# yjtang249/MIPSFusion

Measured on AMD Instinct MI355X. Metric: rays*samples/s per GPU, full optimisation iteration (fwd + bwd + pose+map Adam), 4096 rays x 64 samples, 640x480 RGB-D, higher is better.
Workload: dtype f32; decoder products as 3 x bf16 pieces of each fp32 operand, 6 bf16 MFMAs per product, fp32 accumulate; 1 GPU; BASELINE config 2: FastCaMo-synth apartment_2, 1 active submap per GPU, 4096 rays x 64 samples, hash grid 2^19 x 16 x 2, 620x460 synthetic RGB-D; rays=4096, samples_per_ray=64, hash_size=19, parallelism=single gpu

## Files before the change

include/mipsf.h:

```cpp
#ifndef MIPSF_H
#define MIPSF_H

#include <stdint.h>

#ifdef __cplusplus
extern "C" {
#endif

#define MIPSF_MAX_LEVELS 32
#define MIPSF_ABI_VERSION 2

const char* mipsf_last_error(void);
int mipsf_abi_version(void);
int mipsf_device_cu_count(void);

typedef struct mipsf_grid_meta {
    uint32_t n_levels;
    uint32_t n_features;
    uint32_t log2_hashmap_size;
    uint32_t base_resolution;
    float per_level_scale;
    float log2_per_level_scale;
    uint32_t n_params;
    uint32_t offsets[MIPSF_MAX_LEVELS + 1];
    uint32_t resolutions[MIPSF_MAX_LEVELS];
    float scales[MIPSF_MAX_LEVELS];
} mipsf_grid_meta;

#define MIPSF_SIZE_HASHGRID_BWD_SCRATCH 1
#define MIPSF_SIZE_HASHGRID_COUNTER_WORDS 2
#define MIPSF_SIZE_DECODER_PACKED 3
#define MIPSF_SIZE_DECODER_SAVED 4
#define MIPSF_SIZE_DECODER_DACT 5
#define MIPSF_SIZE_DECODER_WGRAD_PARTIAL 6
#define MIPSF_SIZE_DECODER_PACKED16 7
#define MIPSF_SIZE_DECODER_TILE_WORDS 8
#define MIPSF_SIZE_RENDER_PARTIAL 9
#define MIPSF_SIZE_PLACE_POSE_SCRATCH 10
#define MIPSF_SIZE_POSE_RAYS_SCRATCH 11
#define MIPSF_SIZE_HASHGRID_DET_SCRATCH 12
#define MIPSF_SIZE_DECODER_LIVE_LIST 13
uint64_t mipsf_buffer_size(int which, uint32_t n, uint32_t a, uint32_t b, const mipsf_grid_meta* meta_host);

int mipsf_hashgrid_meta_init(mipsf_grid_meta* meta_host, uint32_t n_levels, uint32_t n_features,
                             uint32_t log2_hashmap_size, uint32_t base_resolution, double per_level_scale);

#define MIPSF_FEAT_AOS 0
#define MIPSF_FEAT_LEVEL_MAJOR 1

int mipsf_hashgrid_fwd(const float* x, const float* params, float* out, float* jac, uint32_t M,
                       const mipsf_grid_meta* meta_host, int layout, void* stream);
int mipsf_hashgrid_dx_from_jac(const float* jac, const float* dout, float* dx, const uint32_t* tile_live, uint32_t M,
                               const mipsf_grid_meta* meta_host, int layout, void* stream);
#define MIPSF_HG_DPARAMS_ZERO 1u
#define MIPSF_HG_ROUTED 2u
#define MIPSF_HG_DETERMINISTIC 4u
#define MIPSF_HG_DET_PIECE 512
#define MIPSF_HG_DET_MAX_ITEMS (1ull << 31)
typedef struct mipsf_hashgrid_bwd_args {
    uint32_t struct_size;
    uint32_t M;
    const float* x;
    const float* params;
    const float* dout;
    float* dparams;
    float* dx;
    float* scratch;
    uint32_t* counters;
    const mipsf_grid_meta* meta;
    int feat_layout;
    uint32_t flags;
} mipsf_hashgrid_bwd_args;
int mipsf_hashgrid_bwd(const mipsf_hashgrid_bwd_args* args_host, void* stream);
int mipsf_hashgrid_route(const float* x, float* scratch, uint32_t M, const mipsf_grid_meta* meta_host, void* stream);
int mipsf_hashgrid_indices(const float* x, uint32_t* idx, uint32_t M, const mipsf_grid_meta* meta_host,
                           void* stream);

int mipsf_freq_fwd(const float* x, float* out, uint32_t M, uint32_t n_dims, uint32_t n_freq, void* stream);
int mipsf_freq_bwd(const float* x, const float* dout, float* dx, uint32_t M, uint32_t n_dims,
                   uint32_t n_freq, void* stream);

typedef struct mipsf_decoder_weights {
    const float* w_pts0; const float* b_pts0;
    const float* w_pts2; const float* b_pts2;
    const float* w_rgb0; const float* b_rgb0;
    const float* w_sdf0; const float* b_sdf0;
    const float* w_sdf2; const float* b_sdf2;
} mipsf_decoder_weights;

typedef struct mipsf_decoder_grads {
    float* w_pts0; float* b_pts0; float* w_pts2; float* b_pts2; float* w_rgb0; float* b_rgb0;
    float* w_sdf0; float* b_sdf0; float* w_sdf2; float* b_sdf2;
} mipsf_decoder_grads;

#define MIPSF_PREC_F32 0
#define MIPSF_PREC_F16X3 1
#define MIPSF_PREC_F16 2
#define MIPSF_PREC_BF16X3 3
#define MIPSF_PREC_BF16X6 4

int mipsf_decoder_pack(const mipsf_decoder_weights* w_host_struct, float* packed, void* stream);
int mipsf_decoder_pack_host(const mipsf_decoder_weights* w_host_ptrs, float* packed_host);
int mipsf_decoder_fwd(const float* packed, const float* feat, int feat_layout, const float* x,
                      const float* embed_pos, int pe_mode, float* out, float* saved, uint32_t M, void* stream);
int mipsf_decoder_fwd_sdf(const float* packed, const float* feat, int feat_layout, const float* x,
                          const float* embed_pos, int pe_mode, float* sdf, uint32_t M, void* stream);
int mipsf_decoder_bwd(const float* packed, const float* feat, int feat_layout, const float* x,
                      const float* embed_pos, int pe_mode, const float* out, const float* dout,
                      const float* saved, float* dfeat, float* dx, float* dembed_pos,
                      const mipsf_decoder_grads* grads_host_struct, float* dact, float* partial,
                      uint32_t M, void* stream);
int mipsf_decoder_bwd_chain(const float* packed, int feat_layout, const float* x, int pe_mode,
                            const float* out, const float* dout, const float* saved, float* dfeat, float* dx,
                            float* dembed_pos, float* dact, uint32_t M, void* stream);
int mipsf_decoder_wgrad(const float* feat, int feat_layout, const float* x, const float* embed_pos, int pe_mode,
                        const float* saved, const float* dact, const mipsf_decoder_grads* grads_host_struct,
                        float* partial, int precision, uint32_t M, void* stream);

int mipsf_decoder_pack16(const mipsf_decoder_weights* w_host_struct, float* packed16, int precision, void* stream);
typedef struct mipsf_decoder_fwd16_args {
    uint32_t struct_size;
    uint32_t M;
    const float* packed16;
    const float* feat;
    const float* x;
    float* out;
    float* saved;
    uint32_t* tile_live_clear;
    int feat_layout;
    int precision;
    int sdf_only;
    int lean_record;
    uint32_t packed16_floats;
} mipsf_decoder_fwd16_args;
int mipsf_decoder_fwd16(const mipsf_decoder_fwd16_args* args_host, void* stream);
#define MIPSF_CHAIN_HEADER_CLEAR 1
#define MIPSF_CHAIN_LEAN_DACT 2
#define MIPSF_CHAIN_BF16X6 4
typedef struct mipsf_decoder_chain16_args {
    uint32_t struct_size;
    uint32_t M;
    const float* packed16;
    const float* x;
    const float* out;
    const float* dout;
    const float* saved;
    float* dfeat;
    float* dx;
    float* dact;
    uint32_t* tile_live;
    int feat_layout;
    int flags;
    uint32_t packed16_floats;
    const uint32_t* live_list;
// ... 63 lines not shown
    double* sums;
    float* draw;
} mipsf_render_fwd_args;
int mipsf_render_fwd(const mipsf_render_fwd_args* args_host, void* stream);
int mipsf_loss_finalize_sums(const double* sums, const mipsf_render_cfg* cfg_host, uint32_t N_total, uint32_t S,
                             float* losses, const float* loss_weights, float* loss_total, void* stream);
typedef struct mipsf_render_bwd_args {
    uint32_t struct_size;
    uint32_t N, S, N_norm;
    const float* raw;
    const float* z_vals;
    const float* target_rgb;
    const float* target_d;
    const uint32_t* counts;
    const float* losses;
    const mipsf_render_cfg* cfg;
    const float* g_losses;
    const float* g_total;
    const float* loss_weights;
    const float* g_rgb;
    const float* g_depth;
    float* draw;
    uint32_t flags;
} mipsf_render_bwd_args;
#define MIPSF_RENDER_BWD_KEEP_IF_UNIT 1u
int mipsf_render_bwd(const mipsf_render_bwd_args* args_host, void* stream);
int mipsf_gather_pose_place_fwd(const float* db, uint64_t n_rows, const int64_t* idx, const float* fixed_poses,
                                const float* rot, const float* trans, uint32_t F, uint32_t K, const int64_t* owner,
                                const float* noise, const float* z_uniform, const float* z_near_offsets,
                                const float* z_near_nodepth, const mipsf_render_cfg* cfg_host, float* d_cam, float* rgb,
                                float* depth, float* z_vals, float* xn, uint32_t* counts, uint32_t N, void* stream);
int mipsf_place_pose_bwd(const float* dxn, const float* z_vals, const mipsf_render_cfg* cfg_host, const float* rot, uint32_t F,
                         uint32_t K, const int64_t* owner, const float* d_cam, float* d_rot, float* d_trans, float* scratch,
                         uint32_t N, uint32_t S, int accumulate, void* stream);
int mipsf_rays_bwd(const float* dxn, const float* z_vals, const mipsf_render_cfg* cfg_host, float* d_rays_o,
                   float* d_rays_d, uint32_t N, uint32_t S, void* stream);
int mipsf_normalise_bwd(const float* dxn, const mipsf_render_cfg* cfg_host, float* dpts, uint32_t M,
                        void* stream);

int mipsf_pose_rays_fwd(const float* db, uint64_t n_rows, const int64_t* idx, const float* fixed_poses,
                        const float* rot, const float* trans, uint32_t F, uint32_t K, const int64_t* owner,
                        float* d_cam, float* rgb, float* depth, float* rays_o, float* rays_d, uint32_t N,
                        void* stream);
#define MIPSF_POSE_MATRIX 0
#define MIPSF_POSE_QUATERNION 1
int mipsf_pose_handover(const float* src, int src_kind, float* rot, float* trans, void* stream);
int mipsf_pose_rays_bwd(const float* g_rays_o, const float* g_rays_d, const float* rot, uint32_t F, uint32_t K,
                        const int64_t* owner, const float* d_cam, float* d_rot, float* d_trans, float* scratch,
                        uint32_t N, int accumulate, void* stream);

int mipsf_adam_step(float* param, float* grad, float* exp_avg, float* exp_avg_sq, uint64_t n, float lr,
                    float beta1, float beta2, float eps, float weight_decay, uint32_t step,
                    const float* hyper_dev, int zero_grad, void* stream);
#define MIPSF_ADAM_MAX_GROUPS 8
int mipsf_adam_advance_n(int32_t* const* step_dev, float* const* hyper_dev, const float* lr, const float* beta1,
                         const float* beta2, uint32_t n_groups, void* stream);

#define MIPSF_ADAM_MAX_TENSORS 16
typedef struct mipsf_adam_tensors {
    uint32_t count;
    float* param[MIPSF_ADAM_MAX_TENSORS];
    float* grad[MIPSF_ADAM_MAX_TENSORS];
    float* exp_avg[MIPSF_ADAM_MAX_TENSORS];
    float* exp_avg_sq[MIPSF_ADAM_MAX_TENSORS];
    uint64_t numel[MIPSF_ADAM_MAX_TENSORS];
} mipsf_adam_tensors;
int mipsf_adam_step_multi(const mipsf_adam_tensors* tensors_host_struct, float lr, float beta1, float beta2,
                          float eps, float weight_decay, uint32_t step, const float* hyper_dev, int zero_grad,
                          void* stream);

#define MIPSF_ADAM_SMALL_MAX_NUMEL 16384
typedef struct mipsf_adam_small {
    uint32_t n_groups, n_tensors;
    int32_t* step_dev[MIPSF_ADAM_MAX_GROUPS];
    float* hyper_dev[MIPSF_ADAM_MAX_GROUPS];
    float lr[MIPSF_ADAM_MAX_GROUPS], beta1[MIPSF_ADAM_MAX_GROUPS], beta2[MIPSF_ADAM_MAX_GROUPS];
    float eps[MIPSF_ADAM_MAX_GROUPS], weight_decay[MIPSF_ADAM_MAX_GROUPS];
    float* param[MIPSF_ADAM_MAX_TENSORS];
    float* grad[MIPSF_ADAM_MAX_TENSORS];
    float* exp_avg[MIPSF_ADAM_MAX_TENSORS];
    float* exp_avg_sq[MIPSF_ADAM_MAX_TENSORS];
    uint32_t numel[MIPSF_ADAM_MAX_TENSORS];
    uint32_t group_of[MIPSF_ADAM_MAX_TENSORS];
} mipsf_adam_small;
int mipsf_adam_step_small(const mipsf_adam_small* desc_host_struct, int zero_grad, void* stream);
#define MIPSF_ADAM_TICKET_WORDS 576
int mipsf_adam_step_all(const mipsf_adam_small* desc_host_struct, int zero_grad, uint32_t* ticket, void* stream);

int mipsf_ro_fitness(const float* raw, uint32_t raw_stride, const float* target_d, float trunc,
                     float* mean_masked, uint32_t P, uint32_t n, void* stream);
int mipsf_ro_fitness_sdf(const float* sdf, const float* target_d, float trunc, float* mean_masked, uint32_t P,
                         uint32_t n, int point_major, void* stream);

#define MIPSF_RO_STATE_FLOATS 32
int mipsf_ro_particles(const float* pst, const float* state, const float* rays_d_cam, const float* target_d,
                       const mipsf_render_cfg* cfg_host, float* xn, float* pst7, uint32_t P, uint32_t n,
                       int point_major, void* stream);
int mipsf_ro_update(const float* mean_masked, const float* pst7, float* state, float sdf_weight, float rescale,
                    uint32_t P, void* stream);

int mipsf_gather_rays(const float* db, uint64_t n_rows, const int64_t* idx, uint32_t N, float* rays7, float* d_cam,
                      float* rgb, float* depth, void* stream);

#ifdef __cplusplus
}
#endif
#endif
```

mipsfusion_amd/_lib.py:

```python
from __future__ import annotations

import ctypes as C
import os
from typing import Optional

import torch

_HERE = os.path.dirname(os.path.abspath(__file__))
LIB_PATH = os.environ.get("MIPSF_LIB") or os.path.join(_HERE, "libmipsf_hip.so")
MAX_LEVELS = 32
FEAT_AOS, FEAT_LEVEL_MAJOR = 0, 1
PREC = {"f32": 0, "f16x3": 1, "f16": 2, "bf16x3": 3, "bf16x6": 4}


class GridMeta(C.Structure):
    _fields_ = [("n_levels", C.c_uint32), ("n_features", C.c_uint32), ("log2_hashmap_size", C.c_uint32),
                ("base_resolution", C.c_uint32), ("per_level_scale", C.c_float),
                ("log2_per_level_scale", C.c_float), ("n_params", C.c_uint32),
                ("offsets", C.c_uint32 * (MAX_LEVELS + 1)), ("resolutions", C.c_uint32 * MAX_LEVELS),
                ("scales", C.c_float * MAX_LEVELS)]


class DecoderWeights(C.Structure):
    _fields_ = [(n, C.c_void_p) for n in ("w_pts0", "b_pts0", "w_pts2", "b_pts2", "w_rgb0", "b_rgb0",
                                          "w_sdf0", "b_sdf0", "w_sdf2", "b_sdf2")]


DecoderGrads = DecoderWeights


class RenderCfg(C.Structure):
    _fields_ = [("n_uniform", C.c_uint32), ("n_near", C.c_uint32), ("perturb", C.c_int), ("use_bound", C.c_int),
                ("bound_min", C.c_double * 3), ("bound_max", C.c_double * 3), ("half_len", C.c_double * 3),
                ("norm_factor", C.c_double), ("trunc", C.c_float), ("sc_factor", C.c_float),
                ("depth_trunc", C.c_float), ("rgb_missing_nonzero", C.c_int), ("emd_w", C.c_float)]


def _args(name, fields):
    cls = type(name, (C.Structure,), {"_fields_": [("struct_size", C.c_uint32)] + fields})

    def new(**kw):
        a = cls()
        a.struct_size = C.sizeof(cls)
        for k, v in kw.items():
            setattr(a, k, v)
        return a
    cls.new = staticmethod(new)
    return cls


_VP, _CU, _CI = C.c_void_p, C.c_uint32, C.c_int
HashgridBwdArgs = _args("HashgridBwdArgs", [("M", _CU), ("x", _VP), ("params", _VP), ("dout", _VP), ("dparams", _VP), ("dx", _VP),
                                            ("scratch", _VP), ("counters", _VP), ("meta", C.POINTER(GridMeta)),
                                            ("feat_layout", _CI), ("flags", _CU)])
DecoderFwd16Args = _args("DecoderFwd16Args", [("M", _CU), ("packed16", _VP), ("feat", _VP), ("x", _VP), ("out", _VP), ("saved", _VP),
                                              ("tile_live_clear", _VP), ("feat_layout", _CI), ("precision", _CI),
                                              ("sdf_only", _CI), ("lean_record", _CI), ("packed16_floats", _CU)])
DecoderChain16Args = _args("DecoderChain16Args", [("M", _CU), ("packed16", _VP), ("x", _VP), ("out", _VP), ("dout", _VP),
                                                  ("saved", _VP), ("dfeat", _VP), ("dx", _VP), ("dact", _VP), ("tile_live", _VP),
                                                  ("feat_layout", _CI), ("flags", _CI), ("packed16_floats", _CU),
                                                  ("live_list", _VP)])
DecoderWgrad16Args = _args("DecoderWgrad16Args", [("M", _CU), ("packed16", _VP), ("feat", _VP), ("x", _VP), ("saved", _VP),
                                                  ("dact", _VP), ("tile_live", _VP), ("grads", C.POINTER(DecoderGrads)),
                                                  ("partial", _VP), ("feat_layout", _CI), ("arithmetic", _CI), ("flags", _CU),
                                                  ("packed16_floats", _CU), ("live_list", _VP)])
RenderFwdArgs = _args("RenderFwdArgs", [("N", _CU), ("S", _CU), ("raw", _VP), ("z_vals", _VP), ("target_rgb", _VP), ("target_d", _VP),
                                        ("counts", _VP), ("cfg", C.POINTER(RenderCfg)), ("rgb", _VP), ("depth", _VP),
                                        ("depth_var", _VP), ("disp", _VP), ("acc", _VP), ("weights", _VP), ("losses", _VP),
                                        ("partial", _VP), ("loss_weights", _VP), ("loss_total", _VP), ("ticket", _VP),
                                        ("sums", _VP), ("draw", _VP)])
RenderBwdArgs = _args("RenderBwdArgs", [("N", _CU), ("S", _CU), ("N_norm", _CU), ("raw", _VP), ("z_vals", _VP), ("target_rgb", _VP),
                                        ("target_d", _VP), ("counts", _VP), ("losses", _VP), ("cfg", C.POINTER(RenderCfg)),
                                        ("g_losses", _VP), ("g_total", _VP), ("loss_weights", _VP), ("g_rgb", _VP),
                                        ("g_depth", _VP), ("draw", _VP), ("flags", _CU)])
RENDER_BWD_KEEP_IF_UNIT = 1

(SIZE_HASHGRID_BWD_SCRATCH, SIZE_HASHGRID_COUNTER_WORDS, SIZE_DECODER_PACKED, SIZE_DECODER_SAVED, SIZE_DECODER_DACT,
 SIZE_DECODER_WGRAD_PARTIAL, SIZE_DECODER_PACKED16, SIZE_DECODER_TILE_WORDS, SIZE_RENDER_PARTIAL, SIZE_PLACE_POSE_SCRATCH,
 SIZE_POSE_RAYS_SCRATCH, SIZE_HASHGRID_DET_SCRATCH, SIZE_DECODER_LIVE_LIST) = range(1, 14)
LIVE_HEADER, LIVE_PAD = 16, 0xFFFFFFFF

HG_DPARAMS_ZERO, HG_ROUTED, HG_DETERMINISTIC = 1, 2, 4
HG_DET_PIECE = 512
HG_DET_MAX_ITEMS = 1 << 31
TILE_ORDER_MAX_M = 1 << 27
WGRAD_LEAN_DACT, WGRAD_DETERMINISTIC = 1, 2


ADAM_MAX_TENSORS = 16


class AdamTensors(C.Structure):
    _fields_ = [("count", C.c_uint32), ("param", C.c_void_p * ADAM_MAX_TENSORS), ("grad", C.c_void_p * ADAM_MAX_TENSORS),
                ("exp_avg", C.c_void_p * ADAM_MAX_TENSORS), ("exp_avg_sq", C.c_void_p * ADAM_MAX_TENSORS),
                ("numel", C.c_uint64 * ADAM_MAX_TENSORS)]


ADAM_MAX_GROUPS = 8
ADAM_SMALL_MAX_NUMEL = 16384


class AdamSmall(C.Structure):
    _fields_ = [("n_groups", C.c_uint32), ("n_tensors", C.c_uint32),
                ("step_dev", C.c_void_p * ADAM_MAX_GROUPS), ("hyper_dev", C.c_void_p * ADAM_MAX_GROUPS),
                ("lr", C.c_float * ADAM_MAX_GROUPS), ("beta1", C.c_float * ADAM_MAX_GROUPS),
                ("beta2", C.c_float * ADAM_MAX_GROUPS), ("eps", C.c_float * ADAM_MAX_GROUPS),
                ("weight_decay", C.c_float * ADAM_MAX_GROUPS),
                ("param", C.c_void_p * ADAM_MAX_TENSORS), ("grad", C.c_void_p * ADAM_MAX_TENSORS),
                ("exp_avg", C.c_void_p * ADAM_MAX_TENSORS), ("exp_avg_sq", C.c_void_p * ADAM_MAX_TENSORS),
                ("numel", C.c_uint32 * ADAM_MAX_TENSORS), ("group_of", C.c_uint32 * ADAM_MAX_TENSORS)]


_P = C.c_void_p
_U32, _U64, _I, _F, _D = C.c_uint32, C.c_uint64, C.c_int, C.c_float, C.c_double

SIGNATURES = {
    "mipsf_last_error": (C.c_char_p, []),
    "mipsf_abi_version": (_I, []),
    "mipsf_device_cu_count": (_I, []),
    "mipsf_buffer_size": (_U64, [_I, _U32, _U32, _U32, C.POINTER(GridMeta)]),
    "mipsf_hashgrid_meta_init": (_I, [C.POINTER(GridMeta), _U32, _U32, _U32, _U32, _D]),
    "mipsf_hashgrid_fwd": (_I, [_P, _P, _P, _P, _U32, C.POINTER(GridMeta), _I, _P]),
    "mipsf_hashgrid_dx_from_jac": (_I, [_P, _P, _P, _P, _U32, C.POINTER(GridMeta), _I, _P]),
    "mipsf_hashgrid_bwd": (_I, [C.POINTER(HashgridBwdArgs), _P]),
    "mipsf_hashgrid_route": (_I, [_P, _P, _U32, C.POINTER(GridMeta), _P]),    "mipsf_hashgrid_indices": (_I, [_P, _P, _U32, C.POINTER(GridMeta), _P]),
    "mipsf_freq_fwd": (_I, [_P, _P, _U32, _U32, _U32, _P]),
    "mipsf_freq_bwd": (_I, [_P, _P, _P, _U32, _U32, _U32, _P]),
    "mipsf_decoder_pack": (_I, [C.POINTER(DecoderWeights), _P, _P]),
    "mipsf_decoder_pack_host": (_I, [C.POINTER(DecoderWeights), _P]),
    "mipsf_decoder_fwd": (_I, [_P, _P, _I, _P, _P, _I, _P, _P, _U32, _P]),
    "mipsf_decoder_fwd_sdf": (_I, [_P, _P, _I, _P, _P, _I, _P, _U32, _P]),
    "mipsf_decoder_bwd": (_I, [_P, _P, _I, _P, _P, _I, _P, _P, _P, _P, _P, _P, C.POINTER(DecoderGrads), _P, _P,
                               _U32, _P]),
    "mipsf_decoder_bwd_chain": (_I, [_P, _I, _P, _I, _P, _P, _P, _P, _P, _P, _P, _U32, _P]),
    "mipsf_decoder_wgrad": (_I, [_P, _I, _P, _P, _I, _P, _P, C.POINTER(DecoderGrads), _P, _I, _U32, _P]),
    "mipsf_decoder_pack16": (_I, [C.POINTER(DecoderWeights), _P, _I, _P]),
    "mipsf_decoder_fwd16": (_I, [C.POINTER(DecoderFwd16Args), _P]),
    "mipsf_decoder_bwd_chain16": (_I, [C.POINTER(DecoderChain16Args), _P]),
    "mipsf_decoder_wgrad16": (_I, [C.POINTER(DecoderWgrad16Args), _P]),
    "mipsf_sample_rays": (_I, [_P, _P, _P, _P, _P, _P, _P, C.POINTER(RenderCfg), _P, _P, _P, _U32, _P]),
    "mipsf_normalise_points": (_I, [_P, C.POINTER(RenderCfg), _P, _U32, _P]),
    "mipsf_render_fwd": (_I, [C.POINTER(RenderFwdArgs), _P]),
    "mipsf_loss_finalize_sums": (_I, [_P, C.POINTER(RenderCfg), _U32, _U32, _P, _P, _P, _P]),
    "mipsf_render_bwd": (_I, [C.POINTER(RenderBwdArgs), _P]),
    "mipsf_gather_pose_place_fwd": (_I, [_P, _U64, _P, _P, _P, _P, _U32, _U32, _P, _P, _P, _P, _P, C.POINTER(RenderCfg), _P, _P,
                                         _P, _P, _P, _P, _U32, _P]),
    "mipsf_place_pose_bwd": (_I, [_P, _P, C.POINTER(RenderCfg), _P, _U32, _U32, _P, _P, _P, _P, _P, _U32, _U32, _I, _P]),
    "mipsf_rays_bwd": (_I, [_P, _P, C.POINTER(RenderCfg), _P, _P, _U32, _U32, _P]),
    "mipsf_normalise_bwd": (_I, [_P, C.POINTER(RenderCfg), _P, _U32, _P]),
    "mipsf_pose_rays_fwd": (_I, [_P, _U64, _P, _P, _P, _P, _U32, _U32, _P, _P, _P, _P, _P, _P, _U32, _P]),
    "mipsf_pose_handover": (_I, [_P, _I, _P, _P, _P]),
    "mipsf_pose_rays_bwd": (_I, [_P, _P, _P, _U32, _U32, _P, _P, _P, _P, _P, _U32, _I, _P]),
    "mipsf_adam_step": (_I, [_P, _P, _P, _P, _U64, _F, _F, _F, _F, _F, _U32, _P, _I, _P]),
    "mipsf_adam_advance_n": (_I, [_P, _P, _P, _P, _P, _U32, _P]),
    "mipsf_adam_step_multi": (_I, [C.POINTER(AdamTensors), _F, _F, _F, _F, _F, _U32, _P, _I, _P]),
    "mipsf_adam_step_small": (_I, [C.POINTER(AdamSmall), _I, _P]),
    "mipsf_adam_step_all": (_I, [C.POINTER(AdamSmall), _I, _P, _P]),
    "mipsf_ro_fitness": (_I, [_P, _U32, _P, _F, _P, _U32, _U32, _P]),
    "mipsf_ro_fitness_sdf": (_I, [_P, _P, _F, _P, _U32, _U32, _I, _P]),
    "mipsf_ro_particles": (_I, [_P, _P, _P, _P, C.POINTER(RenderCfg), _P, _P, _U32, _U32, _I, _P]),
    "mipsf_ro_update": (_I, [_P, _P, _P, _F, _F, _U32, _P]),
    "mipsf_gather_rays": (_I, [_P, _U64, _P, _U32, _P, _P, _P, _P, _P]),
}


SIZE_MCUBES_OFFSET_WORDS, SIZE_MCUBES_WELD_SLOTS, SIZE_MCUBES_WELD_WORDS = 20, 21, 22
MCUBES_BLOCK_CELLS = 4096
McubesArgs = _args("McubesArgs", [("X", _CU), ("Y", _CU), ("Z", _CU), ("isovalue", C.c_float), ("truncation", C.c_float),
                                  ("volume", _VP), ("cases", _VP), ("block_offsets", _VP), ("soup", _VP), ("cell_ids", _VP),
                                  ("capacity_tris", _CU)])
McubesWeldArgs = _args("McubesWeldArgs", [("T", _CU), ("soup", _VP), ("scratch", _VP), ("vertices", _VP), ("faces", _VP),
                                          ("counts", _VP), ("max_rounds", _CU)])
COMPACT_SIGNATURES = {
    "mipsf_decoder_live_compact": (_I, [_P, _U32, _P, _P, _P, _I, _P]),
    "mipsf_hashgrid_dx_from_jac_list": (_I, [_P, _P, _P, _P, _U32, C.POINTER(GridMeta), _I, _P]),
    "mipsf_gather_pose_place_fwd_masked": (_I, [_P, _U64, _P, _P, _P, _P, _U32, _U32, _P, _P, _P, _P, _P, C.POINTER(RenderCfg),
                                                _P, _P, _P, _P, _P, _P, _P, _U32, _P]),
    "mipsf_hashgrid_fwd_masked": (_I, [_P, _P, _P, _P, _P, _U32, _U32, C.POINTER(GridMeta), _I, _P]),
    "mipsf_hashgrid_dx_from_jac_masked": (_I, [_P, _P, _P, _P, _P, _P, _U32, _U32, C.POINTER(GridMeta), _I, _P]),
}

MESH_SIGNATURES = {
    "mipsf_mcubes_count": (_I, [C.POINTER(McubesArgs), _P]),
    "mipsf_mcubes_emit": (_I, [C.POINTER(McubesArgs), _P]),
    "mipsf_mcubes_weld": (_I, [C.POINTER(McubesWeldArgs), _P]),
}


FUSE_KF_FLOATS = 16
FUSE_IN_BOX, FUSE_SEEN = 1, 2


class FusePoints(C.Structure):
# ... 386 lines not shown
```

mipsfusion_amd/csrc/elementwise.hip:

```cpp
#include "common.h"

namespace mipsf {

constexpr float PI_F = 3.14159265358979323846f;
constexpr float HALF_PI_F = 1.57079632679489661923f;

__global__ __launch_bounds__(256) void freq_fwd_kernel(const float* __restrict__ x, float* __restrict__ out,
                                                       uint32_t n, uint32_t n_dims, uint32_t n_freq) {
    const uint32_t t = blockIdx.x * blockDim.x + threadIdx.x;
    if (t >= n) return;
    const uint32_t i = t / n_dims, d = t - i * n_dims;
    const float v = x[t];
    float* o = out + ((size_t)i * n_dims + d) * 2 * n_freq;
    for (uint32_t k = 0; k < n_freq; ++k) {
        const float s = ldexpf(v, (int)k);
        o[2 * k] = sinf(fmaf(s, PI_F, 0.0f));
        o[2 * k + 1] = sinf(fmaf(s, PI_F, HALF_PI_F));
    }
}

__global__ __launch_bounds__(256) void freq_bwd_kernel(const float* __restrict__ x, const float* __restrict__ dout,
                                                       float* __restrict__ dx, uint32_t n, uint32_t n_dims,
                                                       uint32_t n_freq) {
    const uint32_t t = blockIdx.x * blockDim.x + threadIdx.x;
    if (t >= n) return;
    const uint32_t i = t / n_dims, d = t - i * n_dims;
    const float v = x[t];
    const float* g = dout + ((size_t)i * n_dims + d) * 2 * n_freq;
    float acc = 0.f;
    for (uint32_t k = 0; k < n_freq; ++k) {
        const float s = ldexpf(v, (int)k);
        const float fpi = ldexpf(1.0f, (int)k) * PI_F;
        acc = acc + g[2 * k] * (fpi * cosf(fmaf(s, PI_F, 0.0f)));
        acc = acc + g[2 * k + 1] * (fpi * cosf(fmaf(s, PI_F, HALF_PI_F)));
    }
    dx[t] = acc;
}

__global__ __launch_bounds__(256) void normalise_kernel(const float* __restrict__ pts, float* __restrict__ xn,
                                                        uint64_t n3, NormCfg nc) {
    const uint64_t t = (uint64_t)blockIdx.x * blockDim.x + threadIdx.x;
    if (t >= n3) return;
    const int d = (int)(t % 3);
    xn[t] = normalise1(pts[t], nc.sub[d], nc.div[d], nc.norm_factor);
}

__global__ __launch_bounds__(256) void normalise_bwd_kernel(const float* __restrict__ dxn, float* __restrict__ dpts,
                                                            uint64_t n3, NormCfg nc) {
    const uint64_t t = (uint64_t)blockIdx.x * blockDim.x + threadIdx.x;
    if (t >= n3) return;
    const int d = (int)(t % 3);
    dpts[t] = (float)(((double)dxn[t] / nc.norm_factor) / nc.div[d]);
}

struct AdamK {
    float lr_over_bc1, beta1, beta2, one_minus_b1, one_minus_b2, inv_sqrt_bc2, eps, wd;
    const float* dev_hyper;
};

__device__ __forceinline__ AdamK resolve(AdamK k) {
    if (k.dev_hyper) {
        k.lr_over_bc1 = k.dev_hyper[0];
        k.inv_sqrt_bc2 = k.dev_hyper[1];
    }
    return k;
}

__global__ void adam_advance_kernel(int* __restrict__ step, float* __restrict__ hyper, float lr, float beta1,
                                    float beta2) {
    if (threadIdx.x == 0 && blockIdx.x == 0) {
        const int t = step[0] + 1;
        step[0] = t;
        const double bc1 = 1.0 - pow((double)beta1, (double)t);
        const double bc2 = 1.0 - pow((double)beta2, (double)t);
        hyper[0] = (float)((double)lr / bc1);
        hyper[1] = (float)(1.0 / sqrt(bc2));
    }
}

struct AdvanceN {
    int* step[MIPSF_ADAM_MAX_GROUPS];
    float* hyper[MIPSF_ADAM_MAX_GROUPS];
    float lr[MIPSF_ADAM_MAX_GROUPS], beta1[MIPSF_ADAM_MAX_GROUPS], beta2[MIPSF_ADAM_MAX_GROUPS];
    uint32_t n;
};
__global__ void adam_advance_n_kernel(AdvanceN a) {
    const uint32_t i = threadIdx.x;
    if (i >= a.n) return;
    const int t = a.step[i][0] + 1;
    a.step[i][0] = t;
    const double bc1 = 1.0 - pow((double)a.beta1[i], (double)t);
    const double bc2 = 1.0 - pow((double)a.beta2[i], (double)t);
    a.hyper[i][0] = (float)((double)a.lr[i] / bc1);
    a.hyper[i][1] = (float)(1.0 / sqrt(bc2));
}

__device__ __forceinline__ void adam1(float& p, float& g, float& m, float& v, const AdamK& k) {
    float gg = g;
    if (k.wd != 0.f) gg = gg + k.wd * p;
    m = m + (gg - m) * k.one_minus_b1;
    v = v * k.beta2 + (k.one_minus_b2 * gg) * gg;
    const float denom = sqrtf(v) * k.inv_sqrt_bc2 + k.eps;
    p = p - k.lr_over_bc1 * (m / denom);
}

template <bool ZERO>
__global__ __launch_bounds__(256) void adam_kernel(float* __restrict__ p, float* __restrict__ g,
                                                   float* __restrict__ m, float* __restrict__ v, uint64_t n,
                                                   AdamK k_in) {
    const AdamK k = resolve(k_in);
    const uint64_t stride = (uint64_t)gridDim.x * blockDim.x;
    const uint64_t n4 = n / 4;
    float4* p4 = reinterpret_cast<float4*>(p);
    float4* g4 = reinterpret_cast<float4*>(g);
    float4* m4 = reinterpret_cast<float4*>(m);
    float4* v4 = reinterpret_cast<float4*>(v);
    for (uint64_t i = (uint64_t)blockIdx.x * blockDim.x + threadIdx.x; i < n4; i += stride) {
        float4 pp = p4[i], gg = g4[i], mm = m4[i], vv = v4[i];
        adam1(pp.x, gg.x, mm.x, vv.x, k);
        adam1(pp.y, gg.y, mm.y, vv.y, k);
        adam1(pp.z, gg.z, mm.z, vv.z, k);
        adam1(pp.w, gg.w, mm.w, vv.w, k);
        p4[i] = pp;
        m4[i] = mm;
        v4[i] = vv;
        if (ZERO) g4[i] = make_float4(0.f, 0.f, 0.f, 0.f);
    }
    for (uint64_t i = n4 * 4 + (uint64_t)blockIdx.x * blockDim.x + threadIdx.x; i < n; i += stride) {
        float pp = p[i], gg = g[i], mm = m[i], vv = v[i];
        adam1(pp, gg, mm, vv, k);
        p[i] = pp;
        m[i] = mm;
        v[i] = vv;
        if (ZERO) g[i] = 0.f;
    }
}

struct AdamMulti {
    float* p[MIPSF_ADAM_MAX_TENSORS];
    float* g[MIPSF_ADAM_MAX_TENSORS];
    float* m[MIPSF_ADAM_MAX_TENSORS];
    float* v[MIPSF_ADAM_MAX_TENSORS];
    uint64_t n[MIPSF_ADAM_MAX_TENSORS];
};

template <bool ZERO>
__global__ __launch_bounds__(256) void adam_multi_kernel(AdamMulti t, AdamK k_in) {
    const AdamK k = resolve(k_in);
    const int ti = blockIdx.y;
    float *p = t.p[ti], *g = t.g[ti], *m = t.m[ti], *v = t.v[ti];
    const uint64_t n = t.n[ti];
    for (uint64_t i = (uint64_t)blockIdx.x * blockDim.x + threadIdx.x; i < n; i += (uint64_t)gridDim.x * blockDim.x) {
        float pp = p[i], gg = g[i], mm = m[i], vv = v[i];
        adam1(pp, gg, mm, vv, k);
        p[i] = pp, m[i] = mm, v[i] = vv;
        if (ZERO) g[i] = 0.f;
    }
}

template <bool ZERO>
__global__ __launch_bounds__(256) void adam_small_kernel(mipsf_adam_small d) {
    __shared__ float hyp[MIPSF_ADAM_MAX_GROUPS][2];
    if (threadIdx.x < d.n_groups) {
        const uint32_t i = threadIdx.x;
        const int t = d.step_dev[i][0] + 1;
        d.step_dev[i][0] = t;
        const double bc1 = 1.0 - pow((double)d.beta1[i], (double)t);
        const double bc2 = 1.0 - pow((double)d.beta2[i], (double)t);
        const float h0 = (float)((double)d.lr[i] / bc1), h1 = (float)(1.0 / sqrt(bc2));
        hyp[i][0] = h0, hyp[i][1] = h1;
        d.hyper_dev[i][0] = h0, d.hyper_dev[i][1] = h1;
    }
    __syncthreads();
    for (uint32_t ti = 0; ti < d.n_tensors; ++ti) {
        const uint32_t gi = d.group_of[ti];
        AdamK k;
        k.lr_over_bc1 = hyp[gi][0], k.inv_sqrt_bc2 = hyp[gi][1];
        k.beta1 = d.beta1[gi], k.beta2 = d.beta2[gi];
        k.one_minus_b1 = (float)(1.0 - (double)d.beta1[gi]), k.one_minus_b2 = (float)(1.0 - (double)d.beta2[gi]);
        k.eps = d.eps[gi], k.wd = d.weight_decay[gi], k.dev_hyper = nullptr;
        float *p = d.param[ti], *g = d.grad[ti], *m = d.exp_avg[ti], *v = d.exp_avg_sq[ti];
        for (uint32_t i = threadIdx.x; i < d.numel[ti]; i += blockDim.x) {
            float pp = p[i], gg = g[i], mm = m[i], vv = v[i];
            adam1(pp, gg, mm, vv, k);
            p[i] = pp, m[i] = mm, v[i] = vv;
            if (ZERO) g[i] = 0.f;
        }
    }
}

__device__ __forceinline__ double powi(double b, int t) {
    double r = 1.0;
    while (t > 0) {
        if (t & 1) r *= b;
        b *= b;
        t >>= 1;
    }
    return r;
}

__device__ __forceinline__ uint32_t adam_key(float lr, float b1, float b2) {
    return __float_as_uint(lr) ^ (__float_as_uint(b1) * 3u) ^ (__float_as_uint(b2) * 7u);
}

struct AdamAllMap {
    uint32_t blk0[MIPSF_ADAM_MAX_TENSORS + 1];
};

template <bool ZERO>
__global__ __launch_bounds__(256) void adam_all_kernel(mipsf_adam_small d, AdamAllMap map, uint32_t* __restrict__ ticket) {
    __shared__ float hyp[2];
    uint32_t ti = 0;
    while (ti + 1 < d.n_tensors && blockIdx.x >= map.blk0[ti + 1]) ++ti;
    const uint32_t gi = d.group_of[ti];
    float *p = d.param[ti], *g = d.grad[ti], *m = d.exp_avg[ti], *v = d.exp_avg_sq[ti];
    const uint64_t n = d.numel[ti];
    const uint32_t nb = map.blk0[ti + 1] - map.blk0[ti], b = blockIdx.x - map.blk0[ti];
    const uint64_t stride = (uint64_t)nb * 256;
    const bool vec = ((((uintptr_t)p | (uintptr_t)g | (uintptr_t)m | (uintptr_t)v) & 15) == 0);
    const uint64_t n4 = vec ? n / 4 : 0;
    float4* p4 = reinterpret_cast<float4*>(p);
    float4* g4 = reinterpret_cast<float4*>(g);
    float4* m4 = reinterpret_cast<float4*>(m);
    float4* v4 = reinterpret_cast<float4*>(v);
    uint64_t i = (uint64_t)b * 256 + threadIdx.x;
    float4 pp, gg, mm, vv;
    if (i < n4) pp = p4[i], gg = g4[i], mm = m4[i], vv = v4[i];
    uint32_t* nexth = ticket + 16u * 33u + 4u * gi;
    if (threadIdx.x == 0) {
        const int t = d.step_dev[gi][0] + 1;
        const uint32_t tag = nexth[0];
        const float h0 = __uint_as_float(nexth[1]), h1 = __uint_as_float(nexth[2]);
        if (tag == (uint32_t)t && nexth[3] == adam_key(d.lr[gi], d.beta1[gi], d.beta2[gi])) {
            hyp[0] = h0, hyp[1] = h1;
        } else {
            const double bc1 = 1.0 - powi((double)d.beta1[gi], t);
            const double bc2 = 1.0 - powi((double)d.beta2[gi], t);
            hyp[0] = (float)((double)d.lr[gi] / bc1), hyp[1] = (float)(1.0 / sqrt(bc2));
        }
    }
    __syncthreads();
    AdamK k;
    k.lr_over_bc1 = hyp[0], k.inv_sqrt_bc2 = hyp[1];
    k.beta1 = d.beta1[gi], k.beta2 = d.beta2[gi];
    k.one_minus_b1 = (float)(1.0 - (double)d.beta1[gi]), k.one_minus_b2 = (float)(1.0 - (double)d.beta2[gi]);
    k.eps = d.eps[gi], k.wd = d.weight_decay[gi], k.dev_hyper = nullptr;
    if (threadIdx.x == 0) {
        const uint32_t sub = blockIdx.x & 31u;
        const uint32_t n_sub = (gridDim.x - sub + 31u) / 32u;
        bool last = false;
        if (__hip_atomic_fetch_add(ticket + 16u * (1u + sub), 1u, __ATOMIC_RELAXED, __HIP_MEMORY_SCOPE_AGENT) == n_sub - 1) {
            __hip_atomic_store(ticket + 16u * (1u + sub), 0u, __ATOMIC_RELAXED, __HIP_MEMORY_SCOPE_AGENT);
            const uint32_t n_master = gridDim.x < 32u ? gridDim.x : 32u;
            last = __hip_atomic_fetch_add(ticket, 1u, __ATOMIC_RELAXED, __HIP_MEMORY_SCOPE_AGENT) == n_master - 1;
        }
        if (last) {
            for (uint32_t q = 0; q < d.n_groups; ++q) {
                const int t = d.step_dev[q][0] + 1;
                d.step_dev[q][0] = t;
                const double b1 = (double)d.beta1[q], b2 = (double)d.beta2[q];
                d.hyper_dev[q][0] = (float)((double)d.lr[q] / (1.0 - powi(b1, t)));
                d.hyper_dev[q][1] = (float)(1.0 / sqrt(1.0 - powi(b2, t)));
                uint32_t* nx = ticket + 16u * 33u + 4u * q;
                nx[1] = __float_as_uint((float)((double)d.lr[q] / (1.0 - powi(b1, t + 1))));
                nx[2] = __float_as_uint((float)(1.0 / sqrt(1.0 - powi(b2, t + 1))));
                nx[3] = adam_key(d.lr[q], d.beta1[q], d.beta2[q]);
                nx[0] = (uint32_t)(t + 1);
            }
            __hip_atomic_store(ticket, 0u, __ATOMIC_RELAXED, __HIP_MEMORY_SCOPE_AGENT);
        }
    }
    if (i < n4) {
        adam1(pp.x, gg.x, mm.x, vv.x, k);
        adam1(pp.y, gg.y, mm.y, vv.y, k);
        adam1(pp.z, gg.z, mm.z, vv.z, k);
        adam1(pp.w, gg.w, mm.w, vv.w, k);
        p4[i] = pp, m4[i] = mm, v4[i] = vv;
        if (ZERO) g4[i] = make_float4(0.f, 0.f, 0.f, 0.f);
    }
    for (uint64_t r = i + stride; r < n4; r += stride) {
        float4 p1 = p4[r], g1 = g4[r], m1 = m4[r], v1 = v4[r];
        asm volatile("" : "+v"(p1.x), "+v"(g1.x), "+v"(m1.x), "+v"(v1.x));
        adam1(p1.x, g1.x, m1.x, v1.x, k);
        adam1(p1.y, g1.y, m1.y, v1.y, k);
        adam1(p1.z, g1.z, m1.z, v1.z, k);
        adam1(p1.w, g1.w, m1.w, v1.w, k);
        p4[r] = p1, m4[r] = m1, v4[r] = v1;
        if (ZERO) g4[r] = make_float4(0.f, 0.f, 0.f, 0.f);
    }
    for (uint64_t q = n4 * 4 + (uint64_t)b * 256 + threadIdx.x; q < n; q += stride) {
        float p1 = p[q], g1 = g[q], m1 = m[q], v1 = v[q];
        adam1(p1, g1, m1, v1, k);
        p[q] = p1, m[q] = m1, v[q] = v1;
        if (ZERO) g[q] = 0.f;
    }
}

__global__ __launch_bounds__(256) void ro_fitness_kernel(const float* __restrict__ raw, uint32_t stride,
                                                         const float* __restrict__ target_d, float trunc,
                                                         float* __restrict__ out, uint32_t P, uint32_t n,
                                                         uint32_t row_p, uint32_t row_j) {
    const uint32_t wave = (blockIdx.x * blockDim.x + threadIdx.x) / MIPSF_WAVE;
    const uint32_t lane = threadIdx.x & (MIPSF_WAVE - 1);
    if (wave >= P) return;
    float acc = 0.f;
    for (uint32_t j = lane; j < n; j += MIPSF_WAVE) {
        const float s = raw[((size_t)wave * row_p + (size_t)j * row_j) * stride + 3] * trunc;
        acc += (target_d[j] > 0.f) ? fabsf(s) : 0.f;
    }
    acc = wave_sum(acc);
    if (lane == 0) out[wave] = acc / (float)n;
}

}

using namespace mipsf;

extern "C" {

int mipsf_freq_fwd(const float* x, float* out, uint32_t M, uint32_t n_dims, uint32_t n_freq, void* stream) {
    if (M == 0) return 0;
    MIPSF_REQUIRE(x && out, "null pointer");
    const uint32_t n = M * n_dims;
    hipLaunchKernelGGL(freq_fwd_kernel, dim3((n + 255) / 256), dim3(256), 0, (hipStream_t)stream, x, out, n, n_dims,
                       n_freq);
    return check_launch("freq_fwd");
}

int mipsf_freq_bwd(const float* x, const float* dout, float* dx, uint32_t M, uint32_t n_dims, uint32_t n_freq,
                   void* stream) {
    if (M == 0) return 0;
    MIPSF_REQUIRE(x && dout && dx, "null pointer");
    const uint32_t n = M * n_dims;
    hipLaunchKernelGGL(freq_bwd_kernel, dim3((n + 255) / 256), dim3(256), 0, (hipStream_t)stream, x, dout, dx, n,
                       n_dims, n_freq);
    return check_launch("freq_bwd");
}

int mipsf_normalise_points(const float* pts, const mipsf_render_cfg* cfg, float* xn, uint32_t M, void* stream) {
    if (M == 0) return 0;
    MIPSF_REQUIRE(pts && cfg && xn, "null pointer");
    const uint64_t n3 = (uint64_t)M * 3;
    hipLaunchKernelGGL(normalise_kernel, dim3((uint32_t)((n3 + 255) / 256)), dim3(256), 0, (hipStream_t)stream, pts,
                       xn, n3, make_norm(*cfg));
    return check_launch("normalise_points");
}
// ... 11 lines not shown
                       const float* dev_hyper) {
    AdamK k;
    const double bc1 = 1.0 - pow((double)beta1, (double)(step ? step : 1));
    const double bc2 = 1.0 - pow((double)beta2, (double)(step ? step : 1));
    k.lr_over_bc1 = (float)((double)lr / bc1);
    k.beta1 = beta1;
    k.beta2 = beta2;
    k.one_minus_b1 = (float)(1.0 - (double)beta1);
    k.one_minus_b2 = (float)(1.0 - (double)beta2);
    k.inv_sqrt_bc2 = (float)(1.0 / sqrt(bc2));
    k.eps = eps;
    k.wd = weight_decay;
    k.dev_hyper = dev_hyper;
    return k;
}

int mipsf_adam_advance_n(int32_t* const* step_dev, float* const* hyper_dev, const float* lr, const float* beta1,
                         const float* beta2, uint32_t n_groups, void* stream) {
    if (n_groups == 0) return 0;
    MIPSF_REQUIRE(step_dev && hyper_dev && lr && beta1 && beta2, "null pointer");
    MIPSF_REQUIRE(n_groups <= MIPSF_ADAM_MAX_GROUPS, "at most %d groups per call", MIPSF_ADAM_MAX_GROUPS);
    AdvanceN a;
    a.n = n_groups;
    for (uint32_t i = 0; i < n_groups; ++i) {
        MIPSF_REQUIRE(step_dev[i] && hyper_dev[i], "null pointer in group %u", i);
        a.step[i] = step_dev[i], a.hyper[i] = hyper_dev[i], a.lr[i] = lr[i], a.beta1[i] = beta1[i], a.beta2[i] = beta2[i];
    }
    hipLaunchKernelGGL(adam_advance_n_kernel, dim3(1), dim3(64), 0, (hipStream_t)stream, a);
    return check_launch("adam_advance_n");
}

int mipsf_adam_step(float* param, float* grad, float* exp_avg, float* exp_avg_sq, uint64_t n, float lr, float beta1,
                    float beta2, float eps, float weight_decay, uint32_t step, const float* hyper_dev,
                    int zero_grad, void* stream) {
    if (n == 0) return 0;
    MIPSF_REQUIRE(param && grad && exp_avg && exp_avg_sq, "null pointer");
    MIPSF_REQUIRE(step >= 1 || hyper_dev, "step must be >= 1 (or hyper_dev given)");
    MIPSF_REQUIRE((((uintptr_t)param | (uintptr_t)grad | (uintptr_t)exp_avg | (uintptr_t)exp_avg_sq) & 15) == 0,
                  "adam buffers must be 16-byte aligned");
    const AdamK k = make_adam(lr, beta1, beta2, eps, weight_decay, step, hyper_dev);
    uint64_t want = (n / 4 + 255) / 256;
    uint32_t blocks = (uint32_t)(want < 1 ? 1 : (want > 2048 ? 2048 : want));
    if (zero_grad)
        hipLaunchKernelGGL(adam_kernel<true>, dim3(blocks), dim3(256), 0, (hipStream_t)stream, param, grad, exp_avg,
                           exp_avg_sq, n, k);
    else
        hipLaunchKernelGGL(adam_kernel<false>, dim3(blocks), dim3(256), 0, (hipStream_t)stream, param, grad, exp_avg,
                           exp_avg_sq, n, k);
    return check_launch("adam_step");
}

int mipsf_adam_step_multi(const mipsf_adam_tensors* t, float lr, float beta1, float beta2, float eps,
                          float weight_decay, uint32_t step, const float* hyper_dev, int zero_grad, void* stream) {
    MIPSF_REQUIRE(t != nullptr, "null tensor table");
    if (t->count == 0) return 0;
    MIPSF_REQUIRE(t->count <= MIPSF_ADAM_MAX_TENSORS, "too many tensors (%u)", t->count);
    MIPSF_REQUIRE(step >= 1 || hyper_dev, "step must be >= 1 (or hyper_dev given)");
    AdamMulti a;
    uint64_t nmax = 0;
    for (uint32_t i = 0; i < MIPSF_ADAM_MAX_TENSORS; ++i) {
        const bool live = i < t->count;
        a.p[i] = live ? t->param[i] : nullptr, a.g[i] = live ? t->grad[i] : nullptr;
        a.m[i] = live ? t->exp_avg[i] : nullptr, a.v[i] = live ? t->exp_avg_sq[i] : nullptr;
        a.n[i] = live ? t->numel[i] : 0;
        if (live) {
            MIPSF_REQUIRE(a.p[i] && a.g[i] && a.m[i] && a.v[i], "null pointer in tensor %u", i);
            nmax = a.n[i] > nmax ? a.n[i] : nmax;
        }
    }
    const AdamK k = make_adam(lr, beta1, beta2, eps, weight_decay, step, hyper_dev);
    uint64_t bx = (nmax + 255) / 256;
    if (bx > 64) bx = 64;
    if (bx < 1) bx = 1;
    const dim3 grid((uint32_t)bx, t->count);
    if (zero_grad) hipLaunchKernelGGL(adam_multi_kernel<true>, grid, dim3(256), 0, (hipStream_t)stream, a, k);
    else hipLaunchKernelGGL(adam_multi_kernel<false>, grid, dim3(256), 0, (hipStream_t)stream, a, k);
    return check_launch("adam_step_multi");
}

int mipsf_adam_step_small(const mipsf_adam_small* d, int zero_grad, void* stream) {
    MIPSF_REQUIRE(d, "null descriptor");
    MIPSF_REQUIRE(d->n_groups >= 1 && d->n_groups <= MIPSF_ADAM_MAX_GROUPS, "bad group count %u", d->n_groups);
    MIPSF_REQUIRE(d->n_tensors >= 1 && d->n_tensors <= MIPSF_ADAM_MAX_TENSORS, "bad tensor count %u", d->n_tensors);
    for (uint32_t i = 0; i < d->n_groups; ++i) MIPSF_REQUIRE(d->step_dev[i] && d->hyper_dev[i], "null pointer in group %u", i);
    for (uint32_t i = 0; i < d->n_tensors; ++i) {
        MIPSF_REQUIRE(d->param[i] && d->grad[i] && d->exp_avg[i] && d->exp_avg_sq[i], "null pointer in tensor %u", i);
        MIPSF_REQUIRE(d->numel[i] <= MIPSF_ADAM_SMALL_MAX_NUMEL && d->group_of[i] < d->n_groups, "tensor %u out of range", i);
    }
    if (zero_grad) hipLaunchKernelGGL(adam_small_kernel<true>, dim3(1), dim3(256), 0, (hipStream_t)stream, *d);
    else hipLaunchKernelGGL(adam_small_kernel<false>, dim3(1), dim3(256), 0, (hipStream_t)stream, *d);
    return check_launch("adam_step_small");
}

int mipsf_adam_step_all(const mipsf_adam_small* d, int zero_grad, uint32_t* ticket, void* stream) {
    MIPSF_REQUIRE(d && ticket, "null pointer");
    MIPSF_REQUIRE(d->n_groups >= 1 && d->n_groups <= MIPSF_ADAM_MAX_GROUPS, "bad group count %u", d->n_groups);
    MIPSF_REQUIRE(d->n_tensors >= 1 && d->n_tensors <= MIPSF_ADAM_MAX_TENSORS, "bad tensor count %u", d->n_tensors);
    for (uint32_t i = 0; i < d->n_groups; ++i) MIPSF_REQUIRE(d->step_dev[i] && d->hyper_dev[i], "null pointer in group %u", i);
    AdamAllMap map;
    const int cus = device_cus();
    if (cus <= 0) return 3;
    const uint64_t budget = (uint64_t)cus * 8;
    uint64_t want_all = 0;
    for (uint32_t i = 0; i < d->n_tensors; ++i) want_all += ((uint64_t)d->numel[i] / 4 + 255) / 256 + 1;
    uint32_t blocks = 0;
    for (uint32_t i = 0; i < d->n_tensors; ++i) {
        MIPSF_REQUIRE(d->param[i] && d->grad[i] && d->exp_avg[i] && d->exp_avg_sq[i], "null pointer in tensor %u", i);
        MIPSF_REQUIRE(d->group_of[i] < d->n_groups, "tensor %u: group out of range", i);
        map.blk0[i] = blocks;
        uint64_t want = ((uint64_t)d->numel[i] / 4 + 255) / 256 + 1;
        if (want_all > budget) want = want * budget / want_all;
        blocks += (uint32_t)(want < 1 ? 1 : want);
    }
    for (uint32_t i = d->n_tensors; i <= MIPSF_ADAM_MAX_TENSORS; ++i) map.blk0[i] = blocks;
    if (zero_grad) hipLaunchKernelGGL(adam_all_kernel<true>, dim3(blocks), dim3(256), 0, (hipStream_t)stream, *d, map, ticket);
    else hipLaunchKernelGGL(adam_all_kernel<false>, dim3(blocks), dim3(256), 0, (hipStream_t)stream, *d, map, ticket);
    return check_launch("adam_step_all");
}

int mipsf_ro_fitness(const float* raw, uint32_t raw_stride, const float* target_d, float trunc, float* mean_masked,
                     uint32_t P, uint32_t n, void* stream) {
    if (P == 0) return 0;
    MIPSF_REQUIRE(raw && target_d && mean_masked, "null pointer");
    MIPSF_REQUIRE(raw_stride >= 4, "raw_stride must cover the sdf column");
    const uint32_t threads = P * MIPSF_WAVE;
    hipLaunchKernelGGL(ro_fitness_kernel, dim3((threads + 255) / 256), dim3(256), 0, (hipStream_t)stream, raw,
                       raw_stride, target_d, trunc, mean_masked, P, n, n, 1u);
    return check_launch("ro_fitness");
}

int mipsf_ro_fitness_sdf(const float* sdf, const float* target_d, float trunc, float* mean_masked, uint32_t P,
                         uint32_t n, int point_major, void* stream) {
    if (P == 0) return 0;
    MIPSF_REQUIRE(sdf && target_d && mean_masked, "null pointer");
    const uint32_t threads = P * MIPSF_WAVE;
    hipLaunchKernelGGL(ro_fitness_kernel, dim3((threads + 255) / 256), dim3(256), 0, (hipStream_t)stream, sdf - 3, 1u,
                       target_d, trunc, mean_masked, P, n, point_major ? 1u : n, point_major ? P : 1u);
    return check_launch("ro_fitness");
}

}
```

mipsfusion_amd/csrc/hashgrid.hip:

```cpp
#include "common.h"
#include "launch.h"
#include "decoder_layout.h"

namespace mipsf {

constexpr uint32_t P1 = 2654435761u;
constexpr uint32_t P2 = 805459861u;
constexpr int HG_BLOCK = 256;

struct Cell {
    uint32_t c[3];
    float f[3];
};

__device__ __forceinline__ Cell locate(const float* __restrict__ x, uint32_t i, float scale) {
    Cell r;
#pragma unroll
    for (int d = 0; d < 3; ++d) {
        const float pos = fmaf(scale, x[3 * (size_t)i + d], 0.5f);
        const float fl = floorf(pos);
        r.c[d] = (uint32_t)(int)fl;
        r.f[d] = pos - fl;
    }
    return r;
}

template <int MODE>
__device__ __forceinline__ uint32_t corner_index(uint32_t cx, uint32_t cy, uint32_t cz, uint32_t res,
                                                 uint32_t size) {
    if (MODE == 0) {
        uint32_t idx = cx + cy * res + cz * res * res;
        if (idx >= size) {
            idx -= size;
            if (idx >= size) idx %= size;
        }
        return idx;
    }
    const uint32_t h = cx ^ (cy * P1) ^ (cz * P2);
    return MODE == 1 ? (h & (size - 1u)) : (h % size);
}

__host__ __device__ inline bool level_is_hashed(uint32_t res, uint32_t size) {
    uint64_t stride = 1;
    for (int d = 0; d < 3; ++d) {
        if (stride > size) break;
        stride *= res;
        stride &= 0xFFFFFFFFull;
    }
    return size < stride;
}

__device__ __forceinline__ int decode_level(uint32_t n_levels, uint32_t nchunk, uint32_t& chunk) {
    const uint32_t b = blockIdx.x;
    const uint32_t xcd = b & 7u;
    const uint32_t j = b >> 3;
    const uint32_t slot = j / nchunk;
    chunk = j - slot * nchunk;
    const uint32_t nslots = (n_levels + 7u) / 8u;
    return (int)(xcd + 8u * (nslots - 1u - slot));
}

template <int MODE>
__device__ __forceinline__ void corner_indices_m(const Cell& cell, uint32_t res, uint32_t size, uint32_t idx[8]) {
#pragma unroll
    for (int c = 0; c < 8; ++c) {
        idx[c] = corner_index<MODE>(cell.c[0] + (c & 1), cell.c[1] + ((c >> 1) & 1), cell.c[2] + ((c >> 2) & 1),
                                    res, size);
    }
}

__device__ __forceinline__ int level_mode(uint32_t res, uint32_t size) {
    if (!level_is_hashed(res, size)) return 0;
    return (size & (size - 1u)) == 0u ? 1 : 2;
}

__device__ __forceinline__ void corner_indices(int mode, const Cell& cell, uint32_t res, uint32_t size,
                                               uint32_t idx[8]) {
    if (mode == 0) corner_indices_m<0>(cell, res, size, idx);
    else if (mode == 1) corner_indices_m<1>(cell, res, size, idx);
    else corner_indices_m<2>(cell, res, size, idx);
}

__device__ __forceinline__ void corner_weights(const Cell& cell, float w[8]) {
#pragma unroll
// ... 27 lines not shown
        s1 = s1 + wgt * (v[right].y - v[left].y);
    }
}

__device__ __forceinline__ bool ray_wants_dx(const uint32_t* __restrict__ ray_mask, uint32_t S, uint32_t i) {
    return ray_mask == nullptr || ray_mask[S == 64u ? i >> 6 : i / S] != 0u;
}

template <int LAYOUT, bool JAC>
__global__ __launch_bounds__(HG_BLOCK) void hashgrid_fwd_kernel(const float* __restrict__ x,
                                                                const float2* __restrict__ table,
                                                                float* __restrict__ out, float* __restrict__ jac,
                                                                uint32_t M, GridLevels g, uint32_t nchunk,
                                                                const uint32_t* __restrict__ ray_mask, uint32_t S) {
    uint32_t chunk;
    const int level = decode_level(g.n_levels, nchunk, chunk);
    if (level >= (int)g.n_levels) return;
    const uint32_t i = chunk * HG_BLOCK + threadIdx.x;
    if (i >= M) return;

    const uint32_t off = g.offsets[level];
    const uint32_t size = g.offsets[level + 1] - off;
    const uint32_t res = g.res[level];
    const Cell cell = locate(x, i, g.scale[level]);
    uint32_t idx[8];
    corner_indices(level_mode(res, size), cell, res, size, idx);
    float w[8];
    corner_weights(cell, w);
    const float2* lvl = table + off;
    float2 v[8];
#pragma unroll
    for (int c = 0; c < 8; ++c) v[c] = lvl[idx[c]];
    float a0 = 0.f, a1 = 0.f;
#pragma unroll
    for (int c = 0; c < 8; ++c) {
        a0 = fmaf(w[c], v[c].x, a0);
        a1 = fmaf(w[c], v[c].y, a1);
    }
    typedef float f32x2_t __attribute__((ext_vector_type(2)));
    f32x2_t* dst = reinterpret_cast<f32x2_t*>(out + feat_index<LAYOUT>(i, level, M, g.n_levels));
    __builtin_nontemporal_store(f32x2_t{a0, a1}, dst);
    if (JAC && ray_wants_dx(ray_mask, S, i)) {
        f32x2_t* j2 = reinterpret_cast<f32x2_t*>(jac) + (size_t)level * 3 * M + i;
#pragma unroll
        for (int d = 0; d < 3; ++d) {
            float s0, s1;
            level_jacobian(cell, v, g.scale[level], d, s0, s1);
            __builtin_nontemporal_store(f32x2_t{s0, s1}, j2 + (size_t)d * M);
        }
    }
}

constexpr int SC_BLOCK = 1024;
#ifndef MIPSF_SC_PLANAR
#define MIPSF_SC_PLANAR 1
#endif
#if MIPSF_SC_PLANAR
#define SC_ACC0(e) (e)
#define SC_ACC1(e) (sc_plane1 + (e))
#else
#define SC_ACC0(e) (2 * (e))
#define SC_ACC1(e) (2 * (e) + 1)
#endif
#ifndef MIPSF_RT_BLOCK
#define MIPSF_RT_BLOCK 512
#endif
constexpr int RT_BLOCK = MIPSF_RT_BLOCK;
#ifndef MIPSF_SC_MAX_SLICE
#define MIPSF_SC_MAX_SLICE 8192
#endif
constexpr uint32_t SC_MAX_SLICE = MIPSF_SC_MAX_SLICE;
#ifndef MIPSF_SC_SLICE_LOG2
#define MIPSF_SC_SLICE_LOG2 13
#endif
constexpr uint32_t SC_SLICE_LOG2 = MIPSF_SC_SLICE_LOG2;
#ifndef MIPSF_SC_PART
#define MIPSF_SC_PART 24576
#endif
#ifndef MIPSF_SC_PART_DENSE
#define MIPSF_SC_PART_DENSE 8192
#endif
#ifndef MIPSF_SC_RUN
#define MIPSF_SC_RUN 4
#endif
#ifndef MIPSF_SC_SKIP_ZERO
#define MIPSF_SC_SKIP_ZERO 1
#endif
constexpr uint32_t SC_PART = MIPSF_SC_PART;
constexpr uint32_t SC_PART_DENSE = MIPSF_SC_PART_DENSE;
constexpr uint32_t SC_PART_MIN = SC_PART < SC_PART_DENSE ? SC_PART : SC_PART_DENSE;
constexpr uint32_t SC_RUN = MIPSF_SC_RUN;
constexpr uint32_t SC_ROUTE_UNR = 4;
constexpr uint32_t SC_MAX_NS = 512;
constexpr uint32_t SC_MAX_BINS = 8192;
#ifndef MIPSF_SC_MASKED_MAX_M
#define MIPSF_SC_MASKED_MAX_M (1u << 24)
#endif
constexpr uint32_t SC_MASKED_MAX_M = MIPSF_SC_MASKED_MAX_M;

struct ScatterPlan {
    uint32_t n_levels;
    uint32_t n_slices[MIPSF_MAX_LEVELS];
    uint32_t slice_entries[MIPSF_MAX_LEVELS];
    uint32_t slice_shift[MIPSF_MAX_LEVELS];
    uint32_t bin0[MIPSF_MAX_LEVELS + 1];
    uint32_t n_bins;
    uint32_t max_items;
    uint32_t max_slice;
    uint32_t dense_bins;
    uint32_t fresh;
    uint32_t fold_launch;
    uint32_t w_count, w_arrive, w_first, w_parts, w_nitems, w_items;
    uint64_t w_records, w_partial, w_end;
};

static ScatterPlan make_plan(const GridLevels& g, uint32_t M) {
    ScatterPlan p = {};
    p.n_levels = g.n_levels;
    uint32_t bins = 0;
    for (uint32_t l = 0; l < g.n_levels; ++l) {
        const uint32_t size = g.offsets[l + 1] - g.offsets[l];
        const bool one = size <= SC_MAX_SLICE;
        const uint32_t ns = one ? 1u : (size + (1u << SC_SLICE_LOG2) - 1) >> SC_SLICE_LOG2;
        p.n_slices[l] = ns;
        p.slice_entries[l] = one ? size : (1u << SC_SLICE_LOG2);
        p.slice_shift[l] = one ? 31u : SC_SLICE_LOG2;
        p.bin0[l] = bins;
        bins += ns;
    }
    p.bin0[g.n_levels] = bins;
    p.n_bins = bins;
    for (uint32_t l = 0; l < g.n_levels; ++l) {
        if (level_is_hashed(g.res[l], g.offsets[l + 1] - g.offsets[l])) break;
        p.dense_bins = p.bin0[l + 1];
    }
    for (uint32_t l = 0; l < g.n_levels; ++l) p.max_slice = p.slice_entries[l] > p.max_slice ? p.slice_entries[l] : p.max_slice;
    const uint64_t max_records = 8ull * g.n_levels * M;
    p.max_items = (uint32_t)((max_records + SC_PART_MIN - 1) / SC_PART_MIN) + bins;
    uint64_t w = 0;
    p.w_count = (uint32_t)w, w += bins;
    p.w_nitems = (uint32_t)w, w += 4;
    p.w_arrive = (uint32_t)w, w += bins;
    p.w_first = (uint32_t)w, w += bins;
    p.w_parts = (uint32_t)w, w += bins;
    w = (w + 3) / 4 * 4;
    p.w_items = (uint32_t)w;
    w = (w + 15) / 16 * 16;
    p.w_records = w, w += (uint64_t)bins * M;
    w = (w + 15) / 16 * 16;
    p.w_partial = w, w += (uint64_t)p.max_items * SC_MAX_SLICE * 2;
    p.w_end = w;
    return p;
}

__global__ void scatter_zero_kernel(uint32_t* __restrict__ ws, uint32_t n) {
    const uint32_t i = blockIdx.x * blockDim.x + threadIdx.x;
    if (i < n) ws[i] = 0u;
}

__device__ __forceinline__ uint32_t ranked_add(uint32_t* cnt, uint32_t s, bool active, bool aggregate) {
    if (!aggregate) return active ? atomicAdd(&cnt[s], 1u) : 0u;
    const uint32_t lane = threadIdx.x & 63u;
    uint32_t rank = 0;
    unsigned long long todo = __ballot(active);
    while (todo) {
        const int leader = __ffsll((long long)todo) - 1;
        const uint32_t s0 = (uint32_t)__shfl((int)s, leader, 64);
        const unsigned long long m = __ballot(active && s == s0);
        uint32_t b = 0;
        if ((int)lane == leader) b = atomicAdd(&cnt[s0], (uint32_t)__popcll(m));
        b = (uint32_t)__shfl((int)b, leader, 64);
        if (active && s == s0) rank = b + (uint32_t)__popcll(m & ((1ull << lane) - 1ull));
        todo &= ~m;
    }
    return rank;
}

__device__ __forceinline__ void route_groups_general(int mode, const Cell& cell, uint32_t res, uint32_t size,
                                                     uint32_t shift, uint32_t (&s)[8], uint32_t (&m)[8]) {
    uint32_t idx[8];
    corner_indices(mode, cell, res, size, idx);
#pragma unroll
    for (int c = 0; c < 8; ++c) s[c] = idx[c] >> shift;
#pragma unroll
    for (int c = 0; c < 8; ++c) {
        bool first = true;
        uint32_t mm = 0;
#pragma unroll
        for (int k = 0; k < 8; ++k) {
            if (k < c) first = first && (s[k] != s[c]);
            mm |= (s[k] == s[c]) ? (1u << k) : 0u;
        }
        m[c] = first ? mm : 0u;
    }
}

// ... 233 lines not shown
    RT_MARK(5);
    __syncthreads();
    RT_MARK(6);
#pragma unroll
    for (uint32_t u = 0; u < SC_ROUTE_UNR; ++u) {
        const uint32_t i = mine[u];
#pragma unroll
        for (int q = 0; q < 8; ++q) {
            if (q == 4 && !__any(mp[u][1] != 0u)) break;
            const uint32_t m = (mp[u][q >> 2] >> (8 * (q & 3))) & 0xffu;
            if (m) {
                const uint32_t sl = (sp[u][q >> 1] >> (16 * (q & 1))) & 0xffffu;
                const uint32_t rk = (rp[u][q >> 1] >> (16 * (q & 1))) & 0xffffu;
                if (MIPSF_SC_STAGE) {
                    const uint32_t p = lstart[sl] + rk;
                    if (p < STAGE_CAP) {
                        stage[p] = masked ? (i | (m << 24)) : i;
                        continue;
                    }
                }
                rec[(size_t)(bin0 + sl) * M + base[sl] + rk] = masked ? (i | (m << 24)) : i;
            }
        }
    }
    RT_MARK(7);
    if (MIPSF_SC_STAGE) {
        __syncthreads();
        RT_MARK(8);
        const uint32_t wave = threadIdx.x >> 6, lane = threadIdx.x & 63u;
        for (uint32_t q = wave; q < ns; q += RT_BLOCK / 64) {
            const uint32_t n = cnt[q], src = lstart[q];
            uint32_t* dstp = rec + (size_t)(bin0 + q) * M + base[q];
            for (uint32_t p = lane; p < n && src + p < STAGE_CAP; p += 64) dstp[p] = stage[src + p];
        }
    }
#ifdef MIPSF_RT_TRACE
    RT_MARK(9);
    for (int q = 2; q < 9; ++q) tr_acc[q] += tr_t[q + 1] - tr_t[q];
    ++tr_levels;
#endif
    }
#ifdef MIPSF_RT_TRACE
    if ((threadIdx.x & 63u) == 0u) {
        unsigned long long* tr = reinterpret_cast<unsigned long long*>(ws + plan.w_end + 64) + (size_t)(blockIdx.x * (RT_BLOCK / 64) + (threadIdx.x >> 6)) * 10;
        for (int q = 0; q < 9; ++q) tr[q] = tr_acc[q];
        tr[9] = (unsigned long long)(group | (tr_levels << 8));
    }
#endif
}
__device__ __forceinline__ uint32_t part_of(const ScatterPlan& plan, uint32_t bin) {
    return bin < plan.dense_bins ? SC_PART_DENSE : SC_PART;
}

#ifndef MIPSF_SC_PUBLISH_WT
#define MIPSF_SC_PUBLISH_WT 1
#endif

template <bool AGENT>
__device__ __forceinline__ float2 fold_entry(const float2* p2, uint32_t parts, float2 cur) {
    float2 a = make_float2(0.f, 0.f);
    for (uint32_t q = 0; q < parts; q += 8) {
        float2 v[8];
#pragma unroll
        for (uint32_t k = 0; k < 8; ++k) {
            v[k] = make_float2(0.f, 0.f);
            if (q + k < parts) {
                if (AGENT) {
                    const unsigned long long u = __hip_atomic_load(
                        reinterpret_cast<const unsigned long long*>(p2 + (size_t)(q + k) * SC_MAX_SLICE), __ATOMIC_RELAXED,
                        __HIP_MEMORY_SCOPE_AGENT);
                    v[k] = make_float2(__uint_as_float((uint32_t)u), __uint_as_float((uint32_t)(u >> 32)));
                } else {
                    v[k] = p2[(size_t)(q + k) * SC_MAX_SLICE];
                }
            }
        }
#pragma unroll
        for (uint32_t k = 0; k < 8; ++k) a.x += v[k].x, a.y += v[k].y;
    }
    cur.x += a.x, cur.y += a.y;
    return cur;
}

template <int LAYOUT>
__device__ __forceinline__ void scatter_item(const float* __restrict__ x, const float* __restrict__ dout,
                                             float* __restrict__ dparams, uint32_t M, const GridLevels& g,
                                             const ScatterPlan& plan, uint32_t* __restrict__ ws, uint32_t* __restrict__ cw,
                                             uint32_t* sh_flag, double* __restrict__ acc,
                                             const uint4 desc, const uint32_t item_index) {
    const uint32_t item = desc.x;
    const uint32_t sc_plane1 = plan.max_slice;
    (void)sc_plane1;
    const uint32_t bin = item & 0xffffu, part = item >> 16;
    const bool single = desc.z == 1u;
    uint32_t level = 0;
    while (level + 1 < plan.n_levels && bin >= plan.bin0[level + 1]) ++level;
    const uint32_t slice = bin - plan.bin0[level];
    const uint32_t off = g.offsets[level];
    const uint32_t size = g.offsets[level + 1] - off;
    const uint32_t se = plan.slice_entries[level];
    const uint32_t begin = slice * se;
    const uint32_t count = begin + se <= size ? se : size - begin;
    const uint32_t res = g.res[level];
    const float scale = g.scale[level];
    const uint32_t n_rec_bin = desc.y;
    const uint32_t r0 = part * part_of(plan, bin);
    const uint32_t n_rec = n_rec_bin - r0 < part_of(plan, bin) ? n_rec_bin - r0 : part_of(plan, bin);
    const uint32_t* __restrict__ rec = ws + plan.w_records + (size_t)bin * M + r0;

    {
#if MIPSF_SC_PLANAR
        for (uint32_t e = threadIdx.x; e < count; e += SC_BLOCK) acc[SC_ACC0(e)] = 0.0, acc[SC_ACC1(e)] = 0.0;
#else
        double2* z = reinterpret_cast<double2*>(acc);
        for (uint32_t e = threadIdx.x; e < count; e += SC_BLOCK) z[e] = make_double2(0.0, 0.0);
#endif
    }
    float2* dst = reinterpret_cast<float2*>(dparams) + off + begin;
    constexpr uint32_t FL = SC_MAX_SLICE / SC_BLOCK;
    float2 cur[FL];
    if (single && !plan.fresh) {
#pragma unroll
        for (uint32_t k = 0; k < FL; ++k) {
            const uint32_t e = threadIdx.x + k * SC_BLOCK;
            cur[k] = e < count ? dst[e] : make_float2(0.f, 0.f);
        }
    }
    __syncthreads();

    const int mode = level_mode(res, size);
    const bool masked = M <= SC_MASKED_MAX_M;
    uint32_t cc[3] = {0u, 0u, 0u};
    float sum[8][2];
    bool open = false;
    auto flush = [&]() {
#ifdef MIPSF_SC_ABL_DENSE_NOATOM
        if (mode == 0) { asm volatile("" :: "v"(sum[0][0]), "v"(sum[7][1])); return; }
#endif
        Cell cell;
        cell.c[0] = cc[0], cell.c[1] = cc[1], cell.c[2] = cc[2];
        uint32_t idx[8];
        corner_indices(mode, cell, res, size, idx);
        uint32_t hit = 0;
#pragma unroll
        for (int c = 0; c < 8; ++c) {
            idx[c] -= begin;
            hit |= (idx[c] < count) ? (1u << c) : 0u;
        }
        if (mode == 0) {
#pragma unroll
            for (int c = 0; c < 8; ++c) {
                if (hit >> c & 1u) {
                    atomicAdd(&acc[SC_ACC0(idx[c])], (double)sum[c][0]);
                    atomicAdd(&acc[SC_ACC1(idx[c])], (double)sum[c][1]);
                }
            }
            return;
        }
        while (hit) {
            const int c = __ffs((int)hit) - 1;
            hit &= hit - 1u;
            uint32_t e = idx[0];
            float v0 = sum[0][0], v1 = sum[0][1];
#pragma unroll
            for (int k = 1; k < 8; ++k) {
                e = (c == k) ? idx[k] : e;
                v0 = (c == k) ? sum[k][0] : v0;
                v1 = (c == k) ? sum[k][1] : v1;
            }
            atomicAdd(&acc[SC_ACC0(e)], (double)v0);
            atomicAdd(&acc[SC_ACC1(e)], (double)v1);
        }
    };
    if (mode != 0) {
        constexpr int UD = 4;
        for (uint32_t r = threadIdx.x; r < n_rec; r += UD * SC_BLOCK) {
            uint32_t si[UD];
            float px[UD][3];
            float2 pg[UD];
#pragma unroll
            for (int u = 0; u < UD; ++u) {
                const uint32_t q = r + u * SC_BLOCK;
                si[u] = rec[q < n_rec ? q : n_rec - 1];
            }
#pragma unroll
            for (int u = 0; u < UD; ++u) {
                const uint32_t ii = masked ? (si[u] & 0xffffffu) : si[u];
#ifdef MIPSF_SC_ABL_NOGATHER
                px[u][0] = (float)(ii & 1023u) * (1.0f / 1024.0f), px[u][1] = (float)((ii >> 10) & 1023u) * (1.0f / 1024.0f);
                px[u][2] = (float)((ii >> 5) & 1023u) * (1.0f / 1024.0f);
                pg[u] = make_float2(1e-3f, 2e-3f);
#else
                px[u][0] = x[3 * (size_t)ii], px[u][1] = x[3 * (size_t)ii + 1], px[u][2] = x[3 * (size_t)ii + 2];
                pg[u] = *reinterpret_cast<const float2*>(dout + feat_index<LAYOUT>(ii, level, M, g.n_levels));
#endif
            }
#pragma unroll
            for (int u = 0; u < UD; ++u) {
                if (r + u * SC_BLOCK >= n_rec) break;
                Cell cell;
#pragma unroll
                for (int d = 0; d < 3; ++d) {
                    const float pos = fmaf(scale, px[u][d], 0.5f);
                    const float fl = floorf(pos);
// ... 27 lines not shown
                            const float wgt = (cell.f[0] * wy) * wz;
                            atomicAdd(&acc[SC_ACC0(e)], (double)(wgt * gy.x));
                            atomicAdd(&acc[SC_ACC1(e)], (double)(wgt * gy.y));
                        }
                    }
                    continue;
                }
                while (hit) {
                    const int c = __ffs((int)hit) - 1;
                    hit &= hit - 1u;
                    const uint32_t cx = cell.c[0] + (c & 1), cy = cell.c[1] + ((c >> 1) & 1), cz = cell.c[2] + ((c >> 2) & 1);
                    const uint32_t e = (mode == 1 ? corner_index<1>(cx, cy, cz, res, size) : corner_index<2>(cx, cy, cz, res, size)) - begin;
                    float wgt = (c & 1) ? cell.f[0] : 1.0f - cell.f[0];
                    wgt = wgt * ((c & 2) ? cell.f[1] : 1.0f - cell.f[1]);
                    wgt = wgt * ((c & 4) ? cell.f[2] : 1.0f - cell.f[2]);
                    atomicAdd(&acc[SC_ACC0(e)], (double)(wgt * gy.x));
                    atomicAdd(&acc[SC_ACC1(e)], (double)(wgt * gy.y));
                }
            }
        }
    } else {
    constexpr int UNR = (int)SC_RUN;
    const uint32_t chunk_id = threadIdx.x;
    for (uint32_t r = chunk_id * SC_RUN; r < n_rec; r += SC_BLOCK * SC_RUN) {
        const uint32_t re = r + SC_RUN < n_rec ? r + SC_RUN : n_rec;
        uint32_t si[UNR];
        float px[UNR][3];
        float2 pg[UNR];
#pragma unroll
        for (int u = 0; u < UNR; ++u) {
            si[u] = rec[r + u < re ? r + u : re - 1];
            si[u] = masked ? (si[u] & 0xffffffu) : si[u];
        }
#pragma unroll
        for (int u = 0; u < UNR; ++u) {
            const uint32_t ii = si[u];
#ifdef MIPSF_SC_ABL_DENSE_NOGATHER
            px[u][0] = (float)(ii & 4095u) * (1.0f / 4096.0f), px[u][1] = (float)((ii >> 6) & 4095u) * (1.0f / 4096.0f);
            px[u][2] = (float)((ii >> 12) & 63u) * (1.0f / 64.0f);
            pg[u] = make_float2(1e-3f, 2e-3f);
#else
            px[u][0] = x[3 * (size_t)ii], px[u][1] = x[3 * (size_t)ii + 1], px[u][2] = x[3 * (size_t)ii + 2];
            pg[u] = *reinterpret_cast<const float2*>(dout + feat_index<LAYOUT>(ii, level, M, g.n_levels));
#endif
        }
#pragma unroll
        for (int u = 0; u < UNR; ++u) {
            if (r + u >= re) break;
            Cell cell;
#pragma unroll
            for (int d = 0; d < 3; ++d) {
                const float pos = fmaf(scale, px[u][d], 0.5f);
                const float fl = floorf(pos);
                cell.c[d] = (uint32_t)(int)fl;
                cell.f[d] = pos - fl;
            }
            const bool same = open && cell.c[0] == cc[0] && cell.c[1] == cc[1] && cell.c[2] == cc[2];
            if (!same) {
#ifndef MIPSF_SC_ABL_DENSE_NOMID
                if (open) flush();
#endif
                cc[0] = cell.c[0], cc[1] = cell.c[1], cc[2] = cell.c[2];
#pragma unroll
                for (int c = 0; c < 8; ++c) sum[c][0] = 0.0f, sum[c][1] = 0.0f;
                open = true;
            }
            const float2 gy = pg[u];
#pragma unroll
            for (int c = 0; c < 8; ++c) {
                float wgt = (c & 1) ? cell.f[0] : 1.0f - cell.f[0];
                wgt = wgt * ((c & 2) ? cell.f[1] : 1.0f - cell.f[1]);
                wgt = wgt * ((c & 4) ? cell.f[2] : 1.0f - cell.f[2]);
                sum[c][0] = sum[c][0] + wgt * gy.x;
                sum[c][1] = sum[c][1] + wgt * gy.y;
            }
        }
        if (open) flush();
        open = false;
    }
    }
    __syncthreads();

    auto a2 = [&](uint32_t e) { return make_double2(acc[SC_ACC0(e)], acc[SC_ACC1(e)]); };
    if (single) {
#pragma unroll
        for (uint32_t k = 0; k < FL; ++k) {
            const uint32_t e = threadIdx.x + k * SC_BLOCK;
            if (e < count) {
                const double2 a = a2(e);
                dst[e] = plan.fresh ? make_float2((float)a.x, (float)a.y) : make_float2(cur[k].x + (float)a.x, cur[k].y + (float)a.y);
            }
        }
    } else {
        float2* part0 = reinterpret_cast<float2*>(reinterpret_cast<float*>(ws) + plan.w_partial);
        float2* pdst = part0 + (size_t)item_index * SC_MAX_SLICE;
        if (plan.fold_launch) {
            for (uint32_t e = threadIdx.x; e < count; e += SC_BLOCK) {
                const double2 a = a2(e);
                pdst[e] = make_float2((float)a.x, (float)a.y);
            }
            return;
        }
        for (uint32_t e = threadIdx.x; e < count; e += SC_BLOCK) {
            const double2 a = a2(e);
#if MIPSF_SC_PUBLISH_WT
            __hip_atomic_store(reinterpret_cast<unsigned long long*>(pdst + e),
                               (unsigned long long)__float_as_uint((float)a.x) | ((unsigned long long)__float_as_uint((float)a.y) << 32),
                               __ATOMIC_RELAXED, __HIP_MEMORY_SCOPE_AGENT);
#else
            pdst[e] = make_float2((float)a.x, (float)a.y);
#endif
        }
        asm volatile("s_waitcnt vmcnt(0)" ::: "memory");
        __syncthreads();
        if (threadIdx.x == 0) {
#if !MIPSF_SC_PUBLISH_WT
            __builtin_amdgcn_fence(__ATOMIC_RELEASE, "agent");
            asm volatile("s_waitcnt vmcnt(0)" ::: "memory");
#endif
            const uint32_t before = __hip_atomic_fetch_add(&cw[plan.w_arrive + bin], 1u, __ATOMIC_RELAXED, __HIP_MEMORY_SCOPE_AGENT);
            const bool last = before == desc.z - 1u;
            if (last) {
                __builtin_amdgcn_fence(__ATOMIC_ACQUIRE, "agent");
                asm volatile("s_waitcnt vmcnt(0)" ::: "memory");
            }
            *sh_flag = last ? 1u : 0u;
        }
        __syncthreads();
        if (*sh_flag == 0u) return;
        const float2* p2 = part0 + (size_t)(item_index - part) * SC_MAX_SLICE;
        for (uint32_t e = threadIdx.x; e < count; e += SC_BLOCK)
            dst[e] = fold_entry<true>(p2 + e, desc.z, plan.fresh ? make_float2(0.f, 0.f) : dst[e]);
        if (threadIdx.x == 0) __hip_atomic_store(&cw[plan.w_arrive + bin], 0u, __ATOMIC_RELAXED, __HIP_MEMORY_SCOPE_AGENT);
    }
}


template <int LAYOUT>
__global__ __launch_bounds__(SC_BLOCK) void hashgrid_scatter_persist_kernel(const float* __restrict__ x,
                                                                           const float* __restrict__ dout,
                                                                           float* __restrict__ dparams, uint32_t M,
                                                                           GridLevels g, ScatterPlan plan,
                                                                           uint32_t* __restrict__ ws,
                                                                           uint32_t* __restrict__ cw) {
    extern __shared__ __attribute__((aligned(16))) double acc[];
    __shared__ uint32_t wtot[16];
    __shared__ uint32_t sh_total, sh_next;
    __shared__ uint4 sh_desc;
    constexpr uint32_t PER = SC_MAX_BINS / SC_BLOCK;
    const uint32_t t = threadIdx.x;
    uint32_t* scnt = reinterpret_cast<uint32_t*>(acc + 2 * (size_t)plan.max_slice);
    uint32_t litm = 0;
#pragma unroll
    for (uint32_t k = 0; k < PER; ++k) {
        const uint32_t b = t * PER + k;
        const uint32_t c = b < plan.n_bins ? cw[plan.w_count + b] : 0u;
        if (b < plan.n_bins) scnt[b] = c;
        litm += (c + part_of(plan, b) - 1) / part_of(plan, b);
    }
    uint32_t oitm;
    {
        uint32_t incl = litm;
#pragma unroll
        for (int d = 1; d < 64; d <<= 1) {
            const uint32_t v = (uint32_t)__shfl_up((int)incl, d, 64);
            incl += (int)(t & 63u) >= d ? v : 0u;
        }
        if ((t & 63u) == 63u) wtot[t >> 6] = incl;
        __syncthreads();
        uint32_t before = 0;
        for (uint32_t q = 0; q < (t >> 6); ++q) before += wtot[q];
        oitm = before + incl - litm;
        if (t == SC_BLOCK - 1) sh_total = before + incl;
    }
    {
        uint32_t first = oitm;
        for (uint32_t k = 0; k < PER; ++k) {
            const uint32_t b = t * PER + k;
            if (b >= plan.n_bins) break;
            const uint32_t parts = (scnt[b] + part_of(plan, b) - 1) / part_of(plan, b);
            cw[plan.w_first + b] = first, cw[plan.w_parts + b] = parts;
            first += parts;
        }
    }
    __syncthreads();
    const uint32_t total = sh_total;
    if (t == 0) sh_next = __hip_atomic_fetch_add(&cw[plan.w_nitems + 1], 1u, __ATOMIC_RELAXED, __HIP_MEMORY_SCOPE_AGENT);
    __syncthreads();
    if (sh_next == gridDim.x - 1) {
        for (uint32_t b = t; b < plan.n_bins; b += SC_BLOCK) cw[plan.w_count + b] = 0u;
    }
    for (;;) {
        __syncthreads();
        if (t == 0) sh_next = __hip_atomic_fetch_add(&cw[plan.w_nitems], 1u, __ATOMIC_RELAXED, __HIP_MEMORY_SCOPE_AGENT);
        __syncthreads();
        const uint32_t i = sh_next;
        if (i >= total) break;
        if (i >= oitm && i < oitm + litm) {
            uint32_t first = oitm;
            for (uint32_t k = 0; k < PER; ++k) {
                const uint32_t b = t * PER + k;
                if (b >= plan.n_bins) break;
                const uint32_t c = scnt[b];
                const uint32_t parts = (c + part_of(plan, b) - 1) / part_of(plan, b);
                if (i >= first && i < first + parts) sh_desc = make_uint4(b | ((i - first) << 16), c, parts, 0u);
                first += parts;
            }
        }
        __syncthreads();
        const uint4 desc = sh_desc;
#ifdef MIPSF_SC_TRACE
        const uint64_t tr_t0 = wall_clock64();
#endif
        scatter_item<LAYOUT>(x, dout, dparams, M, g, plan, ws, cw, &wtot[0], acc, desc, i);
#ifdef MIPSF_SC_TRACE
        __syncthreads();
        if (t == 0) {
            const uint64_t tr_t1 = wall_clock64();
            uint32_t* tr = ws + plan.w_end + 64 + 8 * (size_t)i;
            tr[0] = i, tr[1] = desc.x, tr[2] = desc.y, tr[3] = (uint32_t)tr_t0, tr[4] = (uint32_t)tr_t1;
            tr[5] = __builtin_amdgcn_s_getreg((31 << 11) | 20), tr[6] = blockIdx.x, tr[7] = desc.z;
            if (i == 0) ws[plan.w_end + 63] = total;
        }
#endif
    }
    __syncthreads();
    if (t == 0) {
        if (__hip_atomic_fetch_add(&cw[plan.w_nitems + 2], 1u, __ATOMIC_RELAXED, __HIP_MEMORY_SCOPE_AGENT) == gridDim.x - 1) {
            __hip_atomic_store(&cw[plan.w_nitems], 0u, __ATOMIC_RELAXED, __HIP_MEMORY_SCOPE_AGENT);
            __hip_atomic_store(&cw[plan.w_nitems + 1], 0u, __ATOMIC_RELAXED, __HIP_MEMORY_SCOPE_AGENT);
            __hip_atomic_store(&cw[plan.w_nitems + 2], 0u, __ATOMIC_RELAXED, __HIP_MEMORY_SCOPE_AGENT);
        }
    }
}

__global__ __launch_bounds__(256) void hashgrid_scatter_reduce_kernel(float* __restrict__ dparams, GridLevels g,
                                                                      ScatterPlan plan, const uint32_t* __restrict__ ws,
                                                                      const uint32_t* __restrict__ cw) {
    const uint32_t bin = blockIdx.x;
    const uint32_t parts = cw[plan.w_parts + bin];
    if (parts <= 1) return;
    uint32_t level = 0;
    while (level + 1 < plan.n_levels && bin >= plan.bin0[level + 1]) ++level;
    const uint32_t size = g.offsets[level + 1] - g.offsets[level];
    const uint32_t se = plan.slice_entries[level];
    const uint32_t begin = (bin - plan.bin0[level]) * se;
    const uint32_t count = begin + se <= size ? se : size - begin;
    const uint32_t e = blockIdx.y * 256 + threadIdx.x;
    if (e >= count) return;
    const float2* p2 = reinterpret_cast<const float2*>(reinterpret_cast<const float*>(ws) + plan.w_partial) +
                       (size_t)cw[plan.w_first + bin] * SC_MAX_SLICE + e;
    float2* d = reinterpret_cast<float2*>(dparams) + g.offsets[level] + begin + e;
    *d = fold_entry<false>(p2, parts, plan.fresh ? make_float2(0.f, 0.f) : *d);
}

template <int LAYOUT>
MIPSF_SINGLE_FP32 __global__ __launch_bounds__(HG_BLOCK) void hashgrid_dx_kernel(const float* __restrict__ x,
                                                               const float2* __restrict__ table,
                                                               const float* __restrict__ dout,
                                                               float* __restrict__ dxl, uint32_t M, GridLevels g,
                                                               uint32_t nchunk) {
    uint32_t chunk;
    const int level = decode_level(g.n_levels, nchunk, chunk);
    if (level >= (int)g.n_levels) return;
    const uint32_t i = chunk * HG_BLOCK + threadIdx.x;
    if (i >= M) return;
    const uint32_t off = g.offsets[level];
    const uint32_t size = g.offsets[level + 1] - off;
    const uint32_t res = g.res[level];
    const float scale = g.scale[level];
    const Cell cell = locate(x, i, scale);
    uint32_t idx[8];
    corner_indices(level_mode(res, size), cell, res, size, idx);
    const float2 gy = *reinterpret_cast<const float2*>(dout + feat_index<LAYOUT>(i, level, M, g.n_levels));
    const float2* lvl = table + off;
    float2 v[8];
#pragma unroll
    for (int c = 0; c < 8; ++c) v[c] = lvl[idx[c]];
    float gx[3];
#pragma unroll
    for (int d = 0; d < 3; ++d) {
        float s0, s1;
        level_jacobian(cell, v, scale, d, s0, s1);
        gx[d] = s0 * gy.x + s1 * gy.y;
    }
    float* o = dxl + ((size_t)level * M + i) * 3;
    o[0] = gx[0], o[1] = gx[1], o[2] = gx[2];
}

__global__ __launch_bounds__(256) void hashgrid_dx_reduce_kernel(const float* __restrict__ dxl, float* __restrict__ dx,
                                                                 uint64_t n3, uint32_t L) {
    const uint64_t t = (uint64_t)blockIdx.x * blockDim.x + threadIdx.x;
    if (t >= n3) return;
    float a = 0.f;
    for (uint32_t l = 0; l < L; ++l) a += dxl[(uint64_t)l * n3 + t];
    dx[t] += a;
}

template <int LAYOUT>
MIPSF_SINGLE_FP32 __global__ __launch_bounds__(256) void hashgrid_dx_jac_kernel(const float* __restrict__ jac,
                                                              const float* __restrict__ dout, float* __restrict__ dx,
                                                              uint32_t M, uint32_t L,
                                                              const uint32_t* __restrict__ tiles,
                                                              const uint32_t* __restrict__ live_list,
                                                              const uint32_t* __restrict__ ray_mask, uint32_t S) {
    uint32_t i = blockIdx.x * blockDim.x + threadIdx.x;
    if (live_list != nullptr) {
        if (i >= M || i >= live_list[0]) return;
        i = live_list[MIPSF_LIVE_HEADER + i];
    }
    if (tiles != nullptr) {
        const uint32_t k = i >> 5, cap = mipsf::dl::tl_cap((M + 31u) / 32u);
        uint32_t q = 0, first = 0, total = 0;
#pragma unroll
        for (uint32_t j = 0; j < 8; ++j) {
            const uint32_t n = tiles[64 * j + 32];
            if (k >= total && n != 0u) q = j, first = total;
            total += n;
        }
        if (k >= total) return;
        i = tiles[mipsf::dl::TL_HEADER + q * cap + (k - first)] * 32u + (i & 31u);
    }
    if (i >= M) return;
    if (!ray_wants_dx(ray_mask, S, i)) {
        dx[3 * (size_t)i] = 0.f, dx[3 * (size_t)i + 1] = 0.f, dx[3 * (size_t)i + 2] = 0.f;
        return;
    }
    float a[3] = {0.f, 0.f, 0.f};
    for (uint32_t l = 0; l < L; ++l) {
        const float2* j2 = reinterpret_cast<const float2*>(jac) + (size_t)l * 3 * M + i;
        const float2 gy = *reinterpret_cast<const float2*>(dout + feat_index<LAYOUT>(i, l, M, L));
#pragma unroll
        for (int d = 0; d < 3; ++d) {
            const float2 j = j2[(size_t)d * M];
            a[d] += j.x * gy.x + j.y * gy.y;
        }
// ... 410 lines not shown
    return dx_from_jac(jac, dout, dx, nullptr, live_list, M, meta, layout, stream);
}

}
namespace mipsf {
uint64_t hashgrid_bwd_scratch_floats(const mipsf_grid_meta* meta, uint32_t M, int need_dx) {
    GridLevels g;
    if (to_levels(meta, g)) return 0;
    const ScatterPlan p = make_plan(g, M);
#ifdef MIPSF_SC_TRACE
    return p.w_end + 64 + 8ull * p.max_items + 64;
#endif
#ifdef MIPSF_RT_TRACE
    return p.w_end + 64 + 20ull * (RT_BLOCK / 64) * (route_groups(g.n_levels) * ((M + RT_BLOCK * SC_ROUTE_UNR - 1) / (RT_BLOCK * SC_ROUTE_UNR))) + 64;
#endif
    return p.w_end + (need_dx ? (uint64_t)g.n_levels * M * 3 : 0) + 64;
}
uint64_t hashgrid_counter_words(const mipsf_grid_meta* meta) {
    GridLevels g;
    if (to_levels(meta, g)) return 0;
    return make_plan(g, 1).w_items;
}
}
extern "C" {


#ifdef MIPSF_SC_TRACE
uint64_t mipsf_hashgrid_trace_words(const mipsf_grid_meta* meta, uint32_t M, uint32_t* n_rows, uint32_t* bin0) {
    GridLevels g;
    if (to_levels(meta, g)) return 0;
    const ScatterPlan p = make_plan(g, M);
    *n_rows = p.max_items;
    for (uint32_t l = 0; l <= g.n_levels; ++l) bin0[l] = p.bin0[l];
    return p.w_end + 64;
}
#endif


#ifdef MIPSF_RT_TRACE
uint64_t mipsf_hashgrid_rt_trace_words(const mipsf_grid_meta* meta, uint32_t M, uint32_t* n_rows) {
    GridLevels g;
    if (to_levels(meta, g)) return 0;
    const ScatterPlan p = make_plan(g, M);
    *n_rows = (RT_BLOCK / 64) * route_groups(g.n_levels) * ((M + RT_BLOCK * SC_ROUTE_UNR - 1) / (RT_BLOCK * SC_ROUTE_UNR));
    return p.w_end + 64;
}
#endif

static int check_plan(const ScatterPlan& plan, const GridLevels& g, uint32_t M) {
    MIPSF_REQUIRE(plan.n_bins <= SC_MAX_BINS && plan.n_bins <= 0xffffu, "grid too large: %u table slices", plan.n_bins);
    for (uint32_t l = 0; l < g.n_levels; ++l)
        MIPSF_REQUIRE(plan.n_slices[l] <= SC_MAX_NS, "level %u too large: %u slices", l, plan.n_slices[l]);
    MIPSF_REQUIRE(plan.w_end < (1ull << 32), "batch too large for 32-bit scratch offsets (M = %u)", M);
    MIPSF_REQUIRE(((uint64_t)M + SC_PART_MIN - 1) / SC_PART_MIN < (1u << 16), "batch too large (M = %u)", M);
    return 0;
}

static int launch_route(const float* x, const float* dout, int layout, uint32_t* ws, uint32_t* cw, bool clear, uint32_t M,
                        const GridLevels& g, const ScatterPlan& plan, hipStream_t s) {
    if (clear) {
        const uint32_t nz = plan.w_first;
        hipLaunchKernelGGL(scatter_zero_kernel, dim3((nz + 255) / 256), dim3(256), 0, s, cw, nz);
    }
    const uint32_t rb = route_groups(g.n_levels) * ((M + RT_BLOCK * SC_ROUTE_UNR - 1) / (RT_BLOCK * SC_ROUTE_UNR));
    return with_layout(layout, [&](auto LAY) {
        hipLaunchKernelGGL(scatter_route_kernel<LAY.value>, dim3(rb), dim3(RT_BLOCK), 0, s, x, dout, M, g, plan, ws, cw);
        return check_launch("hashgrid_route");
    });
}

int mipsf_hashgrid_route(const float* x, float* scratch, uint32_t M, const mipsf_grid_meta* meta, void* stream) {
    GridLevels g;
    if (int rc = to_levels(meta, g)) return rc;
    if (M == 0) return 0;
    MIPSF_REQUIRE(x && scratch, "null pointer");
    const ScatterPlan plan = make_plan(g, M);
    if (int rc = check_plan(plan, g, M)) return rc;
    uint32_t* ws = reinterpret_cast<uint32_t*>(scratch);
    return launch_route(x, nullptr, MIPSF_FEAT_AOS, ws, ws, true, M, g, plan, (hipStream_t)stream);
}

static int hashgrid_bwd_impl(const float* x, const float* params, const float* dout, float* dparams, float* dx,
                             float* scratch, uint32_t* counters, uint32_t M, const mipsf_grid_meta* meta, int layout,
                             bool routed, void* stream, bool fresh = false) {
    GridLevels g;
    if (int rc = to_levels(meta, g)) return rc;
    if (M == 0) return 0;
    MIPSF_REQUIRE(x && params && dout && scratch, "null pointer");
    MIPSF_REQUIRE(dparams || dx, "nothing to compute: dparams and dx are both null");
    MIPSF_REQUIRE(layout == MIPSF_FEAT_AOS || layout == MIPSF_FEAT_LEVEL_MAJOR, "bad layout %d", layout);
    hipStream_t s = (hipStream_t)stream;
    ScatterPlan plan = make_plan(g, M);
    plan.fresh = fresh ? 1u : 0u;
    {
        const char* e = getenv("MIPSF_SC_FOLD_LAUNCH");
        plan.fold_launch = (e && e[0] && e[0] != '0') ? 1u : 0u;
    }
    if (int rc = check_plan(plan, g, M)) return rc;
    uint32_t* ws = reinterpret_cast<uint32_t*>(scratch);
    uint32_t* cw = counters ? counters : ws;
    float* dxl = scratch + ((plan.w_end + 15) / 16) * 16;
    if (dparams) {
        if (!routed)
            if (int e = launch_route(x, MIPSF_SC_SKIP_ZERO ? dout : nullptr, layout, ws, cw, counters == nullptr, M, g, plan, s)) return e;
        const uint32_t lds_bytes = plan.max_slice * 16 + plan.n_bins * 4;
        const int cus = device_cus();
        if (cus <= 0) return 3;
        uint32_t per_cu = (160u * 1024u) / (lds_bytes + 256u);
        per_cu = per_cu < 1u ? 1u : (per_cu > 2048u / SC_BLOCK ? 2048u / SC_BLOCK : per_cu);
        const uint32_t want = (uint32_t)cus * per_cu;
        const uint32_t blocks = plan.max_items < want ? plan.max_items : want;
        const int rc = with_layout(layout, [&](auto LAY) {
            constexpr auto kern = hashgrid_scatter_persist_kernel<LAY.value>;
            if (!grant_lds<kern>(lds_bytes)) return lds_refused(lds_bytes);
            hipLaunchKernelGGL(kern, dim3(blocks), dim3(SC_BLOCK), lds_bytes, s, x, dout, dparams, M, g, plan, ws, cw);
            return check_launch("hashgrid_scatter");
        });
        if (rc) return rc;
        if (plan.fold_launch) {
            hipLaunchKernelGGL(hashgrid_scatter_reduce_kernel, dim3(plan.n_bins, (plan.max_slice + 255) / 256), dim3(256), 0, s,
                               dparams, g, plan, ws, cw);
            if (int e = check_launch("hashgrid_scatter_reduce")) return e;
        }
    }
    if (dx) return launch_dx(x, params, dout, dxl, dx, M, g, layout, s);
    return 0;
}

int mipsf_hashgrid_bwd(const mipsf_hashgrid_bwd_args* a, void* stream) {
    MIPSF_REQUIRE(a != nullptr, "null argument block");
    MIPSF_REQUIRE(a->struct_size == sizeof(mipsf_hashgrid_bwd_args), "mipsf_hashgrid_bwd_args: struct_size %u, this library expects %u",
                  a->struct_size, (unsigned)sizeof(mipsf_hashgrid_bwd_args));
    MIPSF_REQUIRE((a->flags & ~(uint32_t)(MIPSF_HG_DPARAMS_ZERO | MIPSF_HG_ROUTED | MIPSF_HG_DETERMINISTIC)) == 0u,
                  "unknown flags 0x%x", a->flags);
    if (a->flags & MIPSF_HG_DETERMINISTIC) {
        MIPSF_REQUIRE(!(a->flags & MIPSF_HG_ROUTED), "MIPSF_HG_DETERMINISTIC with MIPSF_HG_ROUTED: the routed scratch belongs to "
                      "the fast scatter; the deterministic path takes its own scratch (MIPSF_SIZE_HASHGRID_DET_SCRATCH)");
        return hashgrid_bwd_det(a->x, a->params, a->dout, a->dparams, a->dx, a->scratch, a->M, a->meta, a->feat_layout,
                                (a->flags & MIPSF_HG_DPARAMS_ZERO) != 0u, stream);
    }
    return hashgrid_bwd_impl(a->x, a->params, a->dout, a->dparams, a->dx, a->scratch, a->counters, a->M, a->meta, a->feat_layout,
                             (a->flags & MIPSF_HG_ROUTED) != 0u, stream, (a->flags & MIPSF_HG_DPARAMS_ZERO) != 0u);
}

int mipsf_hashgrid_indices(const float* x, uint32_t* idx, uint32_t M, const mipsf_grid_meta* meta, void* stream) {
    GridLevels g;
    if (int rc = to_levels(meta, g)) return rc;
    if (M == 0) return 0;
    MIPSF_REQUIRE(x && idx, "null pointer");
    uint32_t nchunk;
    const uint32_t nb = grid_blocks(M, g.n_levels, nchunk);
    hipLaunchKernelGGL(hashgrid_indices_kernel, dim3(nb), dim3(HG_BLOCK), 0, (hipStream_t)stream, x, idx, M, g,
                       nchunk);
    return check_launch("hashgrid_indices");
}

}
```

mipsfusion_amd/model/scene_rep.py:

```python
import copy

import numpy as np
import os
import torch
import torch.nn as nn

from .. import ops
from .._lib import FEAT_LEVEL_MAJOR
from .decoder import MLP_reg
from .encodings import get_encoder


class _PlaceFn(torch.autograd.Function):

    @staticmethod
    def forward(ctx, rays_o, rays_d, target_d, noise, tables, rc, N, S):
        rays_o, rays_d = ops._f32c(rays_o), ops._f32c(rays_d)
        z_vals, xn, counts = ops.sample_rays(rays_o, rays_d, target_d, noise, tables, rc, N, S)
        ctx.rc, ctx.N, ctx.S = rc, N, S
        ctx.save_for_backward(z_vals)
        ctx.mark_non_differentiable(z_vals, counts)
        ctx.set_materialize_grads(False)
        return z_vals, xn, counts

    @staticmethod
    def backward(ctx, _dz, dxn, _dc):
        if dxn is None:
            return (None,) * 8
        (z_vals,) = ctx.saved_tensors
        d_o, d_d = ops.rays_bwd(ops._f32c(dxn), z_vals, ctx.rc, ctx.N, ctx.S)
        return d_o, d_d, None, None, None, None, None, None


class _NormaliseFn(torch.autograd.Function):

    @staticmethod
    def forward(ctx, pts, rc):
        ctx.rc = rc
        return ops.normalise_points(ops._f32c(pts), rc)

    @staticmethod
    def backward(ctx, dxn):
        return ops.normalise_bwd(ops._f32c(dxn), ctx.rc), None


_ROUTE_AHEAD_MIN_M = 65536
_MAX_QUERY, _QUERY_CHUNK = 1 << 24, 1 << 23


class _QueryFn(torch.autograd.Function):

    @staticmethod
    def forward(ctx, xn, owner, grid_params, ray_mask, *weights):
        xn = ops._f32c(xn)
        M = xn.shape[0]
        meta = owner.embed_fn.meta
        jac = None
        routed = None
        if ctx.needs_input_grad[2] and owner.route_ahead and M >= _ROUTE_AHEAD_MIN_M and not ops.resolve_deterministic(owner.deterministic):
            routed = ops.hashgrid_route_ahead(xn, meta)
        if ctx.needs_input_grad[0]:
            feat, jac = ops.hashgrid_fwd(xn, grid_params.detach(), meta, FEAT_LEVEL_MAJOR, with_jac=True, ray_mask=ray_mask)
        else:
            feat = ops.hashgrid_fwd(xn, grid_params.detach(), meta, FEAT_LEVEL_MAJOR)
        need = any(ctx.needs_input_grad)
        prec = owner.decoder_precision
        if prec == "f16" and need:
            raise RuntimeError('decoder_precision "f16" is forward-only (use "bf16x6", "f16x3" or "f32" when gradients are needed)')
        cache = owner._frozen_pack
        if cache is not None and prec in cache:
            packed, packed16 = cache[prec]
        else:
            if prec == "f32":
                packed, packed16 = ops.decoder_pack(weights), None
            else:
                packed, packed16 = None, ops.decoder_pack16(weights, precision=prec)
            if cache is not None:
                cache[prec] = (packed, packed16)
        lean = bool(need and prec in ops.SPLIT_PRECISIONS and owner.wgrad_precision in ("auto", "stream_" + prec) and owner.lean_record)
        masks_only = bool(need and prec in ops.SPLIT_PRECISIONS and not any(ctx.needs_input_grad[4:]))
        out, saved = ops.decoder_fwd(packed, feat, FEAT_LEVEL_MAJOR, xn, None, M,
                                     save="masks" if masks_only else ("lean" if lean else need), precision=prec, packed16=packed16)
        ctx.lean = lean and not masks_only
        ctx.tile_live = getattr(saved, "mipsf_tile_live", None)
        if packed is None:
            packed = packed16
        ctx.prec = prec
        if routed is not None:
            torch.cuda.current_stream(xn.device).wait_event(routed[1])
        ctx.routed = routed
        ctx.owner, ctx.M, ctx.meta, ctx.has_jac = owner, M, meta, jac is not None
        ctx.ray_mask = ray_mask if jac is not None else None
        ctx.save_for_backward(xn, feat, out, saved, packed, grid_params, *weights, *([jac] if jac is not None else []))
        return out

    @staticmethod
    def backward(ctx, dout):
        xn, feat, out, saved, packed, grid_params, *weights = ctx.saved_tensors
        jac = weights.pop() if ctx.has_jac else None
        need_w = any(ctx.needs_input_grad[4:])
        need_g = ctx.needs_input_grad[2]
        need_x = ctx.needs_input_grad[0]
        if ctx.tile_live is not None:
            saved.mipsf_tile_live = ctx.tile_live
        det = ops.resolve_deterministic(ctx.owner.deterministic)
        direct = ctx.owner.accumulate_param_grads_in_place and all(
            p.is_leaf and not p._backward_hooks for p in (grid_params, *weights))
        grads = None
        if need_w:
            grads = []
            for w, need in zip(weights, ctx.needs_input_grad[4:]):
                if direct and need:
                    if w.grad is None:
                        w.grad = torch.zeros_like(w)
                    grads.append(w.grad)
                else:
                    grads.append(torch.zeros_like(w))
        dfeat, dx, _, tiles = ops.decoder_bwd(packed, feat, FEAT_LEVEL_MAJOR, xn, None, out, ops._f32c(dout), saved, grads,
                                              ctx.M, precision=ctx.prec, packed16=packed if ctx.prec != "f32" else None,
                                              wgrad_precision=("stream_" + ctx.prec) if ctx.lean else ctx.owner.wgrad_precision,
                                              recompute_h1=ctx.lean, return_tiles=True, deterministic=det)
        dparams = None
        fresh_grad = False
        if need_g:
            if direct:
                if grid_params.grad is None:
                    grid_params.grad = torch.zeros_like(grid_params)
                    fresh_grad = True
                dparams = grid_params.grad
            else:
                dparams = torch.zeros_like(grid_params)
        if need_g:
            ops.hashgrid_bwd(xn, grid_params.detach(), dfeat, dparams, ctx.meta, FEAT_LEVEL_MAJOR, None, routed=ctx.routed,
                             dparams_zero=(not direct) or fresh_grad or ctx.owner.grid_grad_is_zero_at_backward, deterministic=det)
            ctx.routed = None
        if need_x:
            ops.hashgrid_dx_from_jac(jac, dfeat, dx, ctx.meta, FEAT_LEVEL_MAJOR, tiles=tiles,
                                     ray_mask=ctx.ray_mask)
        w_out = [None] * len(weights)
        if need_w and not direct:
            w_out = [g if need else None for g, need in zip(grads, ctx.needs_input_grad[4:])]
        return (dx if need_x else None, None, None if direct else dparams, None, *w_out)


class _RenderFn(torch.autograd.Function):
    fuse_backward = os.environ.get("MIPSF_RENDER_FUSE_BWD", "1") != "0"

    @staticmethod
    def forward(ctx, raw, z_vals, target_rgb, target_d, counts, rc, N, S, train, loss_w=None, share_of=None):
        raw = ops._f32c(raw)
        total = None
        ctx.n_norm = None
        ctx.draw, ctx.draw_stale = None, False
        if train and share_of is not None:
            rgb, depth, var, disp, acc, _, losses, total, ctx.n_norm = ops.render_fwd(
                raw, z_vals, target_rgb, target_d, counts, rc, N, S, train, loss_weights=loss_w, share_of=share_of)
        elif train and loss_w is not None:
            if ctx.needs_input_grad[0] and S <= ops.RENDER_DRAW_MAX_S and _RenderFn.fuse_backward:
                rgb, depth, var, disp, acc, _, losses, total, ctx.draw = ops.render_fwd(
                    raw, z_vals, target_rgb, target_d, counts, rc, N, S, train, loss_weights=loss_w, want_draw=True)
            else:
                rgb, depth, var, disp, acc, _, losses, total = ops.render_fwd(raw, z_vals, target_rgb, target_d, counts, rc, N,
                                                                              S, train, loss_weights=loss_w)
        else:
            rgb, depth, var, disp, acc, _, losses = ops.render_fwd(raw, z_vals, target_rgb, target_d, counts, rc, N, S,
                                                                   train)
        ctx.rc, ctx.N, ctx.S, ctx.train = rc, N, S, train
        ctx.save_for_backward(raw, z_vals, target_rgb, target_d, counts, losses, loss_w if total is not None else None)
        ctx.mark_non_differentiable(var, disp, acc)
        ctx.set_materialize_grads(False)
        if total is not None:
            return rgb, depth, var, disp, acc, losses, total.reshape(())
        if train:
            return rgb, depth, var, disp, acc, losses
        return rgb, depth, var, disp, acc

    @staticmethod
    def backward(ctx, g_rgb, g_depth, _gv, _gd, _ga, g_losses=None, g_total=None):
        raw, z_vals, target_rgb, target_d, counts, losses, loss_w = ctx.saved_tensors
        g_rgb = ops._f32c(g_rgb) if g_rgb is not None else None
        g_depth = ops._f32c(g_depth) if g_depth is not None else None
        g_total = ops._f32c(g_total).reshape(1) if (g_total is not None and loss_w is not None) else None
        if ctx.draw is not None and not ctx.draw_stale and g_total is not None and g_losses is None and g_rgb is None and g_depth is None:
            one = ops.unit_grad(raw.device)
            if g_total.data_ptr() == one.data_ptr() and one._version == 0:
                return ctx.draw, None, None, None, None, None, None, None, None, None, None
            ctx.draw_stale = True
            draw = ops.render_bwd(raw, z_vals, target_rgb, target_d, counts, losses, ctx.rc, None, None, None, ctx.N, ctx.S,
                                  g_total=g_total, loss_weights=loss_w, keep_draw=ctx.draw)
            return draw, None, None, None, None, None, None, None, None, None, None
        if ctx.train and g_losses is None and g_total is None:
            g_losses = torch.zeros(8, dtype=torch.float32, device=raw.device)
        draw = ops.render_bwd(raw, z_vals, target_rgb, target_d, counts, losses, ctx.rc,
                              ops._f32c(g_losses) if (ctx.train and g_losses is not None) else None, g_rgb, g_depth,
                              ctx.N, ctx.S, g_total=g_total, loss_weights=loss_w, n_norm=ctx.n_norm)
        return draw, None, None, None, None, None, None, None, None, None, None


class JointEncoding(nn.Module):
    def __init__(self, config, bound_box, coords_norm_factor):
        super().__init__()
        self.config = config
        self.bounding_box = bound_box
        self.coords_norm_factor = coords_norm_factor
        self._bound64 = torch.as_tensor(bound_box).detach().to("cpu", torch.float64).tolist()
        self._half64 = torch.as_tensor(coords_norm_factor).detach().to("cpu", torch.float64).reshape(-1).tolist()
        self.accumulate_param_grads_in_place = False
        self.grid_grad_is_zero_at_backward = False
        self.deterministic = None
        self.decoder_precision = "bf16x6"
        self.wgrad_precision = "auto"
        self.lean_record = True
        self.route_ahead = False
        self.mask_fixed_rays = os.environ.get("MIPSF_NO_DX_MASK", "0") != "1"
        self.ray_share_reduce = None
        self._frozen_pack = None
        self._tables = {}
# ... 221 lines not shown
```

mipsfusion_amd/ops.py:

```python
from __future__ import annotations

import ctypes as C
import os
from typing import Optional

import torch

from . import _lib
from ._lib import FEAT_AOS, FEAT_LEVEL_MAJOR, check, dptr, lib, stream_ptr

DECODER_PARAM_ORDER = ("pts_linear.0.weight", "pts_linear.0.bias", "pts_linear.2.weight", "pts_linear.2.bias",
                       "rgb_linear.0.weight", "rgb_linear.0.bias", "sdf_linear.0.weight", "sdf_linear.0.bias",
                       "sdf_linear.2.weight", "sdf_linear.2.bias")
_DEC_FIELDS = ("w_pts0", "b_pts0", "w_pts2", "b_pts2", "w_rgb0", "b_rgb0", "w_sdf0", "b_sdf0", "w_sdf2", "b_sdf2")
_DEC_SHAPES = ((128, 51), (128,), (128, 128), (128,), (3, 115), (3,), (128, 96), (128,), (5, 128), (5,))


PROFILE = None


class _timed:
    def __init__(self, name, stream=None):
        self.name, self.stream = name, stream

# ... 73 lines not shown
                                                        C.byref(meta), layout, stream_ptr()), "hashgrid_dx_from_jac_list")
        return
    with _timed("hashgrid_dx"):
        check(lib().mipsf_hashgrid_dx_from_jac(dptr(jac), dptr(dout), dptr(dx), dptr(tiles, torch.int32), M,
                                               C.byref(meta), layout, stream_ptr()), "hashgrid_dx_from_jac")


_SIDE_STREAMS = {}
SKIP_ZERO_TILES = os.environ.get("MIPSF_NO_TILE_SKIP", "0") != "1"
_LAST_TILE_LIVE = None
COMPACT_LIVE = os.environ.get("MIPSF_NO_COMPACT", "0") != "1"


def last_live_tile_share() -> Optional[float]:
    if _LAST_TILE_LIVE is None:
        return None
    buf, M, compacted = _LAST_TILE_LIVE
    if compacted:
        return float(buf[1].item()) / max(1, (M + 31) // 32)
    counts = buf[32:512:64].cpu()
    return float(counts.sum().item()) / max(1, (M + 31) // 32)


_LAST_SCATTER_DOUT = None


def last_live_record_share() -> Optional[float]:
    if _LAST_SCATTER_DOUT is None:
        return None
    d = _LAST_SCATTER_DOUT.reshape(-1, 2)
    return float(((d[:, 0] != 0) | (d[:, 1] != 0)).float().mean().item())


def side_stream(device) -> "torch.cuda.Stream":
    key = torch.device(device).index if torch.device(device).index is not None else torch.cuda.current_device()
    if key not in _SIDE_STREAMS:
        _SIDE_STREAMS[key] = torch.cuda.Stream(device=key)
    return _SIDE_STREAMS[key]


def hashgrid_route_ahead(x, meta):
    M = x.shape[0]
    n = _lib.buffer_size(_lib.SIZE_HASHGRID_BWD_SCRATCH, M, 0, 0, meta)
    scratch = torch.empty(n, dtype=torch.float32, device=x.device)
    main, side = torch.cuda.current_stream(x.device), side_stream(x.device)
    side.wait_stream(main)
    with _timed("hashgrid_route", side):
        check(lib().mipsf_hashgrid_route(dptr(x), dptr(scratch), M, C.byref(meta), C.c_void_p(side.cuda_stream)),
              "hashgrid_route")
    ev = torch.cuda.Event()
    ev.record(side)
    return scratch, ev


_ZEROED = {}
_lib.KEPT_BLOCK_CACHES.append(_ZEROED)


def _zeroed_words(device, n, tag):
    key = (device.index, stream_ptr(), tag, n)
    buf = _ZEROED.get(key)
    if buf is None:
        buf = _ZEROED[key] = torch.zeros(n, dtype=torch.int32, device=device)
    return buf


_SCATTER_COUNTERS = {}
_lib.KEPT_BLOCK_CACHES.append(_SCATTER_COUNTERS)


def _scatter_counters(device, meta):
    n = _lib.buffer_size(_lib.SIZE_HASHGRID_COUNTER_WORDS, meta=meta)
    key = (device.index, stream_ptr(), n)
    buf = _SCATTER_COUNTERS.get(key)
    if buf is None:
        buf = _SCATTER_COUNTERS[key] = torch.zeros(n, dtype=torch.int32, device=device)
    return buf


LEAN_DACT = not bool(os.environ.get("MIPSF_FULL_DACT"))
HG_DPARAMS_ZERO = 1
HG_ROUTED = 2
HG_DETERMINISTIC = 4
_HG_IGNORE_ZERO_HINT = bool(os.environ.get("MIPSF_HG_IGNORE_ZERO_HINT"))


def hashgrid_bwd(x, params, dout, dparams, meta, layout=FEAT_AOS, dx: Optional[torch.Tensor] = None, routed=None,
                 dparams_zero=False, deterministic=False):
    M = x.shape[0]
    if PROFILE is not None:
        global _LAST_SCATTER_DOUT
        _LAST_SCATTER_DOUT = dout
    a = _lib.HashgridBwdArgs.new(M=M, x=dptr(x), params=dptr(params), dout=dptr(dout), dparams=dptr(dparams),
                                 meta=C.pointer(meta), feat_layout=layout)
    if deterministic:
        if routed is not None:
            torch.cuda.current_stream(x.device).wait_event(routed[1])
        n = _lib.buffer_size(_lib.SIZE_HASHGRID_DET_SCRATCH, M, 1 if dx is not None else 0, 0, meta)
        scratch = torch.empty(n, dtype=torch.float32, device=x.device)
        a.dx, a.scratch = dptr(dx), dptr(scratch)
        a.flags = HG_DETERMINISTIC | (HG_DPARAMS_ZERO if (dparams_zero and not _HG_IGNORE_ZERO_HINT) else 0)
        with _timed("hashgrid_bwd"):
            check(lib().mipsf_hashgrid_bwd(C.byref(a), stream_ptr()), "hashgrid_bwd (deterministic)")
        return
    if routed is not None and dx is None and dparams is not None:
        scratch, ev = routed
        torch.cuda.current_stream(x.device).wait_event(ev)
        a.scratch, a.flags = dptr(scratch), HG_ROUTED
        with _timed("hashgrid_bwd"):
            check(lib().mipsf_hashgrid_bwd(C.byref(a), stream_ptr()), "hashgrid_bwd (routed)")
        return
    n = _lib.buffer_size(_lib.SIZE_HASHGRID_BWD_SCRATCH, M, 1 if dx is not None else 0, 0, meta)
    scratch = torch.empty(n, dtype=torch.float32, device=x.device)
    counters = _scatter_counters(x.device, meta)
    a.dx, a.scratch, a.counters = dptr(dx), dptr(scratch), dptr(counters, torch.int32)
    a.flags = HG_DPARAMS_ZERO if (dparams_zero and not _HG_IGNORE_ZERO_HINT) else 0
    with _timed("hashgrid_bwd"):
        check(lib().mipsf_hashgrid_bwd(C.byref(a), stream_ptr()), "hashgrid_bwd")


def hashgrid_indices(x, meta) -> torch.Tensor:
    M = x.shape[0]
    idx = torch.empty((M, meta.n_levels, 8), dtype=torch.int32, device=x.device)
    check(lib().mipsf_hashgrid_indices(dptr(x), dptr(idx, torch.int32), M, C.byref(meta), stream_ptr()),
          "hashgrid_indices")
    return idx


def resolve_deterministic(flag) -> bool:
    return torch.are_deterministic_algorithms_enabled() if flag is None else bool(flag)


class HashGridFn(torch.autograd.Function):

    @staticmethod
    def forward(ctx, x, params, meta, deterministic=None):
        x = _f32c(x)
        ctx.meta = meta
        ctx.deterministic = deterministic
        if ctx.needs_input_grad[0]:
            out, jac = hashgrid_fwd(x, params.detach(), meta, FEAT_AOS, with_jac=True)
            ctx.save_for_backward(x, params, jac)
            return out
        ctx.save_for_backward(x, params)
        return hashgrid_fwd(x, params.detach(), meta, FEAT_AOS)

    @staticmethod
    def backward(ctx, dout):
        x, params, *jac = ctx.saved_tensors
        dout = _f32c(dout)
        dparams = torch.zeros_like(params) if ctx.needs_input_grad[1] else None
        dx = torch.zeros_like(x) if ctx.needs_input_grad[0] else None
        if dparams is not None:
            hashgrid_bwd(x, params.detach(), dout, dparams, ctx.meta, FEAT_AOS, None, dparams_zero=True,
                         deterministic=resolve_deterministic(ctx.deterministic))
        if dx is not None:
            hashgrid_dx_from_jac(jac[0], dout, dx, ctx.meta, FEAT_AOS)
        return dx, dparams, None, None


class FrequencyFn(torch.autograd.Function):
    @staticmethod
    def forward(ctx, x, n_freq):
        x = _f32c(x)
        ctx.n_freq = n_freq
        ctx.save_for_backward(x)
        M, D = x.shape
        out = torch.empty((M, D * 2 * n_freq), dtype=torch.float32, device=x.device)
        check(lib().mipsf_freq_fwd(dptr(x), dptr(out), M, D, n_freq, stream_ptr()), "freq_fwd")
        return out

    @staticmethod
    def backward(ctx, dout):
        (x,) = ctx.saved_tensors
        M, D = x.shape
        dx = torch.empty_like(x)
        check(lib().mipsf_freq_bwd(dptr(x), dptr(_f32c(dout)), dptr(dx), M, D, ctx.n_freq, stream_ptr()),
              "freq_bwd")
        return dx, None


def _decoder_struct(tensors, cls):
    st = cls()
    for field, t, shape in zip(_DEC_FIELDS, tensors, _DEC_SHAPES):
        if tuple(t.shape) != shape:
            raise RuntimeError(f"decoder tensor {field} has shape {tuple(t.shape)}, expected {shape}")
        setattr(st, field, dptr(t))
    return st


def decoder_pack(weights, packed: Optional[torch.Tensor] = None) -> torch.Tensor:
    dev = weights[0].device
    if packed is None:
        packed = torch.empty(_lib.buffer_size(_lib.SIZE_DECODER_PACKED), dtype=torch.float32, device=dev)
    ws = [w.detach() for w in weights]
    st = _decoder_struct(ws, _lib.DecoderWeights)
    with _timed("decoder_pack"):
        check(lib().mipsf_decoder_pack(C.byref(st), dptr(packed), stream_ptr()), "decoder_pack")
    return packed
# ... 455 lines not shown
    @staticmethod
    def backward(ctx, _g_rgb, _g_depth, _g_z, dxn, _g_counts, _g_wants):
        if dxn is None:
            return (None,) * 11
        rot, owner, d_cam, z_vals = ctx.saved_tensors
        n = _lib.buffer_size(_lib.SIZE_PLACE_POSE_SCRATCH, ctx.N, ctx.F, ctx.K)
        key = (rot.device.index, stream_ptr(), "place", n)
        scratch = _POSE_SCRATCH.get(key)
        if scratch is None:
            scratch = _POSE_SCRATCH[key] = torch.zeros(n, dtype=torch.float32, device=rot.device)
        direct = ctx.params is not None and all(
            p.is_leaf and p.requires_grad and not p._backward_hooks and p.dtype == torch.float32 and p.is_contiguous()
            for p in ctx.params)
        if direct:
            for p in ctx.params:
                if p.grad is None:
                    p.grad = torch.zeros_like(p)
            d_rot, d_trans = ctx.params[0].grad, ctx.params[1].grad
        else:
            d_rot = torch.empty((ctx.K, 4), dtype=torch.float32, device=rot.device)
            d_trans = torch.empty((ctx.K, 3), dtype=torch.float32, device=rot.device)
        with _timed("rays_bwd"):
            check(lib().mipsf_place_pose_bwd(dptr(_f32c(dxn)), dptr(z_vals), C.byref(ctx.rc), dptr(rot), ctx.F, ctx.K,
                                             dptr(owner, torch.int64), dptr(d_cam), dptr(d_rot), dptr(d_trans), dptr(scratch),
                                             ctx.N, ctx.S, 1 if direct else 0, stream_ptr()), "place_pose_bwd")
        if direct:
            return (None,) * 11
        return (d_rot, d_trans) + (None,) * 9


def adam_advance(step_dev, hyper_dev, lr, beta1, beta2):
    adam_advance_n([(step_dev, hyper_dev, lr, beta1, beta2)])


def adam_advance_n(groups):
    n = len(groups)
    steps = (C.c_void_p * n)(*[dptr(g[0], torch.int32) for g in groups])
    hypers = (C.c_void_p * n)(*[dptr(g[1]) for g in groups])
    lr = (C.c_float * n)(*[g[2] for g in groups])
    b1 = (C.c_float * n)(*[g[3] for g in groups])
    b2 = (C.c_float * n)(*[g[4] for g in groups])
    check(lib().mipsf_adam_advance_n(steps, hypers, lr, b1, b2, n, stream_ptr()), "adam_advance_n")


def adam_step(param, grad, exp_avg, exp_avg_sq, lr, beta1, beta2, eps, weight_decay, step, zero_grad=False,
              hyper_dev=None):
    with _timed("adam_step" if param.numel() > (1 << 20) else "adam_step_small"):
        check(lib().mipsf_adam_step(dptr(param), dptr(grad), dptr(exp_avg), dptr(exp_avg_sq), param.numel(), lr,
                                    beta1, beta2, eps, weight_decay, step, dptr(hyper_dev),
                                    1 if zero_grad else 0, stream_ptr()), "adam_step")


def adam_step_multi(params, grads, exp_avgs, exp_avg_sqs, lr, beta1, beta2, eps, weight_decay, step, zero_grad=False,
                    hyper_dev=None):
    for i in range(0, len(params), _lib.ADAM_MAX_TENSORS):
        chunk = slice(i, i + _lib.ADAM_MAX_TENSORS)
        t = _lib.AdamTensors()
        t.count = len(params[chunk])
        for j, (p, g, m, v) in enumerate(zip(params[chunk], grads[chunk], exp_avgs[chunk], exp_avg_sqs[chunk])):
            t.param[j], t.grad[j], t.exp_avg[j], t.exp_avg_sq[j] = dptr(p), dptr(g), dptr(m), dptr(v)
            t.numel[j] = p.numel()
        with _timed("adam_step_small"):
            check(lib().mipsf_adam_step_multi(C.byref(t), lr, beta1, beta2, eps, weight_decay, step,
                                              dptr(hyper_dev), 1 if zero_grad else 0, stream_ptr()),
                  "adam_step_multi")


def adam_step_small(groups, zero_grad=False):
    d = _lib.AdamSmall()
    d.n_groups = len(groups)
    ti = 0
    for gi, (step_dev, hyper_dev, lr, b1, b2, eps, wd, tensors) in enumerate(groups):
        d.step_dev[gi], d.hyper_dev[gi] = dptr(step_dev, torch.int32), dptr(hyper_dev)
        d.lr[gi], d.beta1[gi], d.beta2[gi], d.eps[gi], d.weight_decay[gi] = lr, b1, b2, eps, wd
        for p, g, m, v in tensors:
            d.param[ti], d.grad[ti], d.exp_avg[ti], d.exp_avg_sq[ti] = dptr(p), dptr(g), dptr(m), dptr(v)
            d.numel[ti], d.group_of[ti] = p.numel(), gi
            ti += 1
    d.n_tensors = ti
    with _timed("adam_step_small"):
        check(lib().mipsf_adam_step_small(C.byref(d), 1 if zero_grad else 0, stream_ptr()), "adam_step_small")


def adam_step_all(groups, ticket, zero_grad=False):
    d = _lib.AdamSmall()
    d.n_groups = len(groups)
    ti, dev, big = 0, None, False
    for gi, (step_dev, hyper_dev, lr, b1, b2, eps, wd, tensors) in enumerate(groups):
        d.step_dev[gi], d.hyper_dev[gi] = dptr(step_dev, torch.int32), dptr(hyper_dev)
        d.lr[gi], d.beta1[gi], d.beta2[gi], d.eps[gi], d.weight_decay[gi] = lr, b1, b2, eps, wd
        for p, g, m, v in tensors:
            d.param[ti], d.grad[ti], d.exp_avg[ti], d.exp_avg_sq[ti] = dptr(p), dptr(g), dptr(m), dptr(v)
            d.numel[ti], d.group_of[ti] = p.numel(), gi
            dev, big = p.device, big or p.numel() > (1 << 20)
            ti += 1
    d.n_tensors = ti
    with _timed("adam_step" if big else "adam_step_small"):
        check(lib().mipsf_adam_step_all(C.byref(d), 1 if zero_grad else 0, dptr(ticket, torch.int32), stream_ptr()),
              "adam_step_all")


def ro_fitness(raw, target_d, trunc: float, point_major: bool = False) -> torch.Tensor:
    P, n, stride = raw.shape
    out = torch.empty(P, dtype=torch.float32, device=raw.device)
    if stride == 1:
        check(lib().mipsf_ro_fitness_sdf(dptr(raw), dptr(target_d), trunc, dptr(out), P, n, 1 if point_major else 0,
                                         stream_ptr()), "ro_fitness")
    else:
        check(lib().mipsf_ro_fitness(dptr(raw), stride, dptr(target_d), trunc, dptr(out), P, n, stream_ptr()),
              "ro_fitness")
    return out


RO_STATE_FLOATS = 32


def ro_particles(pst, state, rays_d_cam, target_d, rc, point_major: bool = False):
    P, n = pst.shape[0], rays_d_cam.shape[0]
    xn = torch.empty((P * n, 3), dtype=torch.float32, device=pst.device)
    pst7 = torch.empty((P, 7), dtype=torch.float32, device=pst.device)
    with _timed("ro_particles"):
        check(lib().mipsf_ro_particles(dptr(pst), dptr(state), dptr(rays_d_cam), dptr(target_d), C.byref(rc), dptr(xn),
                                       dptr(pst7), P, n, 1 if point_major else 0, stream_ptr()), "ro_particles")
    return xn, pst7


def ro_update(mean_masked, pst7, state, sdf_weight: float, rescale: float):
    with _timed("ro_update"):
        check(lib().mipsf_ro_update(dptr(mean_masked), dptr(pst7), dptr(state), sdf_weight, rescale,
                                    mean_masked.shape[0], stream_ptr()), "ro_update")


def gather_rays(db, idx, split: bool = False):
    flat = db.reshape(-1, 7)
    N = idx.shape[0]
    dev = flat.device
    if split:
        d_cam = torch.empty((N, 3), dtype=torch.float32, device=dev)
        rgb = torch.empty((N, 3), dtype=torch.float32, device=dev)
        depth = torch.empty((N, 1), dtype=torch.float32, device=dev)
        check(lib().mipsf_gather_rays(dptr(flat), flat.shape[0], dptr(idx, torch.int64), N, None, dptr(d_cam),
                                      dptr(rgb), dptr(depth), stream_ptr()), "gather_rays")
        return d_cam, rgb, depth
    out = torch.empty((N, 7), dtype=torch.float32, device=dev)
    check(lib().mipsf_gather_rays(dptr(flat), flat.shape[0], dptr(idx, torch.int64), N, dptr(out), None, None, None,
                                  stream_ptr()), "gather_rays")
    return out
```

mipsfusion_amd/optim.py:

```python
import torch

from . import _lib, ops


import os

_SPLIT_LAUNCHES = os.environ.get("MIPSF_ADAM_SPLIT", "0") == "1"


class FusedAdam(torch.optim.Optimizer):
    def __init__(self, params, lr=1e-3, betas=(0.9, 0.999), eps=1e-8, weight_decay=0.0, capturable=False):
        super().__init__(params, dict(lr=lr, betas=betas, eps=eps, weight_decay=weight_decay))
        self.capturable = capturable
        self._dev = {}

    def _ensure_state(self, p):
        st = self.state[p]
        if not st:
            st["step"] = 0
            st["exp_avg"] = torch.zeros_like(p, memory_format=torch.contiguous_format)
            st["exp_avg_sq"] = torch.zeros_like(p, memory_format=torch.contiguous_format)
        return st

    @staticmethod
    def _all_small(work):
        n_t = sum(len(live) for _, _, live, _ in work)
        return (len(work) <= _lib.ADAM_MAX_GROUPS and n_t <= _lib.ADAM_MAX_TENSORS and
                all(p.numel() <= _lib.ADAM_SMALL_MAX_NUMEL for _, _, live, _ in work for p in live))

    @torch.no_grad()
    def reset(self):
        tensors = []
        for st in self.state.values():
            if st:
                st["step"] = 0
                tensors += [st["exp_avg"], st["exp_avg_sq"]]
        tensors += [step_dev for step_dev, _ in self._dev.values()]
        by_dtype = {}
        for t in tensors:
            by_dtype.setdefault((t.dtype, t.device), []).append(t)
        for group in by_dtype.values():
            torch._foreach_zero_(group)

    def _sync_steps_from_device(self):
        for gi, (step_dev, _) in self._dev.items():
            n = int(step_dev.item())
            for p in self.param_groups[gi]["params"]:
                if self.state.get(p):
                    self.state[p]["step"] = n

    def state_dict(self):
        self._sync_steps_from_device()
        return super().state_dict()

    @torch.no_grad()
    def load_state_dict(self, state_dict):
        super().load_state_dict(state_dict)
        for st in self.state.values():
            if st and torch.is_tensor(st.get("step")):
                st["step"] = int(st["step"].item())
        for gi, (step_dev, _) in self._dev.items():
            steps = {self.state[p]["step"] for p in self.param_groups[gi]["params"] if self.state.get(p)}
            if len(steps) > 1:
                raise RuntimeError(f"capturable FusedAdam: group {gi} has parameters at different steps {sorted(steps)}")
            if steps:
                step_dev.fill_(steps.pop())

    @torch.no_grad()
    def step(self, closure=None, zero_grad=False):
        loss = None
        if closure is not None:
            with torch.enable_grad():
                loss = closure()
        work = []
        for gi, group in enumerate(self.param_groups):
            b1, b2 = group["betas"]
            live = [p for p in group["params"] if p.grad is not None and p.numel() > 0]
            if not live:
                continue
            for p in live:
                if not p.is_cuda:
                    raise RuntimeError("FusedAdam runs on GPU parameters only (no CPU fallback)")
                self._ensure_state(p)["step"] += 1
            hyper = None
            if self.capturable:
                if len({self.state[p]["step"] for p in live}) > 1:
                    raise RuntimeError(f"capturable FusedAdam: the parameters of group {gi} are at different steps "
                                       "(some had no gradient in an earlier step); use capturable=False for that")
                if gi not in self._dev:
                    dev = live[0].device
                    start = self.state[live[0]]["step"] - 1
                    self._dev[gi] = (torch.full((1,), start, dtype=torch.int32, device=dev),
                                     torch.zeros(2, dtype=torch.float32, device=dev))
                hyper = self._dev[gi][1]
            work.append((gi, group, live, hyper))
        if self.capturable and work and self._all_small(work):
            ops.adam_step_small([(self._dev[gi][0], self._dev[gi][1], group["lr"], group["betas"][0], group["betas"][1],
                                  group["eps"], group["weight_decay"],
                                  [(p.data, p.grad, self.state[p]["exp_avg"], self.state[p]["exp_avg_sq"]) for p in live])
                                 for gi, group, live, _ in work], zero_grad)
            return loss
        n_t = sum(len(live) for _, _, live, _ in work)
        if (self.capturable and work and not _SPLIT_LAUNCHES and len(work) <= _lib.ADAM_MAX_GROUPS and n_t <= _lib.ADAM_MAX_TENSORS and
                all(p.numel() < (1 << 32) and p.is_contiguous() for _, _, live, _ in work for p in live)):
            if getattr(self, "_ticket", None) is None or self._ticket.device != work[0][2][0].device:
                self._ticket = torch.zeros(576, dtype=torch.int32, device=work[0][2][0].device)
            try:
                ops.adam_step_all([(self._dev[gi][0], self._dev[gi][1], group["lr"], group["betas"][0], group["betas"][1],
                                    group["eps"], group["weight_decay"],
                                    [(p.data, p.grad, self.state[p]["exp_avg"], self.state[p]["exp_avg_sq"]) for p in live])
                                   for gi, group, live, _ in work], self._ticket, zero_grad)
            except RuntimeError:
                self._ticket = None
                raise
            return loss
        if self.capturable and work:
            adv = [(self._dev[gi][0], self._dev[gi][1], group["lr"], group["betas"][0], group["betas"][1])
                   for gi, group, _, _ in work]
            for i in range(0, len(adv), 8):
                ops.adam_advance_n(adv[i:i + 8])
        for gi, group, live, hyper in work:
            b1, b2 = group["betas"]
            small = []
            for p in live:
                st = self.state[p]
                if p.numel() < (1 << 18):
                    small.append(p)
                    continue
                ops.adam_step(p.data, p.grad, st["exp_avg"], st["exp_avg_sq"], group["lr"], b1, b2, group["eps"],
                              group["weight_decay"], st["step"], zero_grad, hyper_dev=hyper)
            by_step = {}
            for p in small:
                by_step.setdefault(self.state[p]["step"], []).append(p)
            for step, ps in by_step.items():
                ops.adam_step_multi([p.data for p in ps], [p.grad for p in ps],
                                    [self.state[p]["exp_avg"] for p in ps], [self.state[p]["exp_avg_sq"] for p in ps],
                                    group["lr"], b1, b2, group["eps"], group["weight_decay"], step, zero_grad,
                                    hyper_dev=hyper)
        return loss
```

Baseline: 456.1 million rays*samples/s.

## Fuse hash-grid Adam update into the scatter backward and skip it in step

Adds a fused mode in which the hash-grid backward scatter applies the Adam update directly to the table parameters and moments as it flushes each accumulated slice. The later one-launch Adam step then skips the hash table through a skip mask. This is meant to avoid writing the full dense gradient for the large table and reading it back, along with the separate optimizer pass over it. In exchange it adds strict Python-side bookkeeping: exactly one backward per step(zero_grad=True), and errors if that contract is broken. It also has to visit every table entry during the scatter, including entries that received no gradient records.

Result: slower. 450.6 million rays*samples/s (-1.2%).

```diff
diff --git a/include/mipsf.h b/include/mipsf.h
--- a/include/mipsf.h
+++ b/include/mipsf.h
@@ -55,6 +55,8 @@
 #define MIPSF_HG_DPARAMS_ZERO 1u
 #define MIPSF_HG_ROUTED 2u
 #define MIPSF_HG_DETERMINISTIC 4u
+#define MIPSF_HG_FUSED_ADAM 8u
+#define MIPSF_HG_KEEP_GRAD 16u
 #define MIPSF_HG_DET_PIECE 512
 #define MIPSF_HG_DET_MAX_ITEMS (1ull << 31)
 typedef struct mipsf_hashgrid_bwd_args {
@@ -70,6 +72,15 @@
     const mipsf_grid_meta* meta;
     int feat_layout;
     uint32_t flags;
+    struct {
+        float* params_rw;
+        float* exp_avg;
+        float* exp_avg_sq;
+        const int32_t* step_dev;
+        const uint32_t* ticket;
+        uint32_t group;
+        float lr, beta1, beta2, eps, weight_decay;
+    } adam;
 } mipsf_hashgrid_bwd_args;
 int mipsf_hashgrid_bwd(const mipsf_hashgrid_bwd_args* args_host, void* stream);
 int mipsf_hashgrid_route(const float* x, float* scratch, uint32_t M, const mipsf_grid_meta* meta_host, void* stream);
@@ -299,6 +310,7 @@
     float* exp_avg_sq[MIPSF_ADAM_MAX_TENSORS];
     uint32_t numel[MIPSF_ADAM_MAX_TENSORS];
     uint32_t group_of[MIPSF_ADAM_MAX_TENSORS];
+    uint32_t skip_mask;
 } mipsf_adam_small;
 int mipsf_adam_step_small(const mipsf_adam_small* desc_host_struct, int zero_grad, void* stream);
 #define MIPSF_ADAM_TICKET_WORDS 576
diff --git a/mipsfusion_amd/_lib.py b/mipsfusion_amd/_lib.py
--- a/mipsfusion_amd/_lib.py
+++ b/mipsfusion_amd/_lib.py
@@ -50,9 +50,16 @@
 
 
 _VP, _CU, _CI = C.c_void_p, C.c_uint32, C.c_int
+
+
+class HashgridAdam(C.Structure):
+    _fields_ = [("params_rw", _VP), ("exp_avg", _VP), ("exp_avg_sq", _VP), ("step_dev", _VP), ("ticket", _VP), ("group", _CU),
+                ("lr", C.c_float), ("beta1", C.c_float), ("beta2", C.c_float), ("eps", C.c_float), ("weight_decay", C.c_float)]
+
+
 HashgridBwdArgs = _args("HashgridBwdArgs", [("M", _CU), ("x", _VP), ("params", _VP), ("dout", _VP), ("dparams", _VP), ("dx", _VP),
                                             ("scratch", _VP), ("counters", _VP), ("meta", C.POINTER(GridMeta)),
-                                            ("feat_layout", _CI), ("flags", _CU)])
+                                            ("feat_layout", _CI), ("flags", _CU), ("adam", HashgridAdam)])
 DecoderFwd16Args = _args("DecoderFwd16Args", [("M", _CU), ("packed16", _VP), ("feat", _VP), ("x", _VP), ("out", _VP), ("saved", _VP),
                                               ("tile_live_clear", _VP), ("feat_layout", _CI), ("precision", _CI),
                                               ("sdf_only", _CI), ("lean_record", _CI), ("packed16_floats", _CU)])
@@ -80,7 +87,7 @@
  SIZE_POSE_RAYS_SCRATCH, SIZE_HASHGRID_DET_SCRATCH, SIZE_DECODER_LIVE_LIST) = range(1, 14)
 LIVE_HEADER, LIVE_PAD = 16, 0xFFFFFFFF
 
-HG_DPARAMS_ZERO, HG_ROUTED, HG_DETERMINISTIC = 1, 2, 4
+HG_DPARAMS_ZERO, HG_ROUTED, HG_DETERMINISTIC, HG_FUSED_ADAM, HG_KEEP_GRAD = 1, 2, 4, 8, 16
 HG_DET_PIECE = 512
 HG_DET_MAX_ITEMS = 1 << 31
 TILE_ORDER_MAX_M = 1 << 27
@@ -108,7 +115,8 @@
                 ("weight_decay", C.c_float * ADAM_MAX_GROUPS),
                 ("param", C.c_void_p * ADAM_MAX_TENSORS), ("grad", C.c_void_p * ADAM_MAX_TENSORS),
                 ("exp_avg", C.c_void_p * ADAM_MAX_TENSORS), ("exp_avg_sq", C.c_void_p * ADAM_MAX_TENSORS),
-                ("numel", C.c_uint32 * ADAM_MAX_TENSORS), ("group_of", C.c_uint32 * ADAM_MAX_TENSORS)]
+                ("numel", C.c_uint32 * ADAM_MAX_TENSORS), ("group_of", C.c_uint32 * ADAM_MAX_TENSORS),
+                ("skip_mask", C.c_uint32)]
 
 
 _P = C.c_void_p
diff --git a/mipsfusion_amd/csrc/adam_dev.h b/mipsfusion_amd/csrc/adam_dev.h
--- /dev/null
+++ b/mipsfusion_amd/csrc/adam_dev.h
@@ -0,0 +1,68 @@
+#pragma once
+#include "common.h"
+
+namespace mipsf {
+
+struct AdamK {
+    float lr_over_bc1, beta1, beta2, one_minus_b1, one_minus_b2, inv_sqrt_bc2, eps, wd;
+    const float* dev_hyper;
+};
+
+__device__ __forceinline__ AdamK resolve(AdamK k) {
+    if (k.dev_hyper) {
+        k.lr_over_bc1 = k.dev_hyper[0];
+        k.inv_sqrt_bc2 = k.dev_hyper[1];
+    }
+    return k;
+}
+
+__device__ __forceinline__ void adam1(float& p, float& g, float& m, float& v, const AdamK& k) {
+    float gg = g;
+    if (k.wd != 0.f) gg = gg + k.wd * p;
+    m = m + (gg - m) * k.one_minus_b1;
+    v = v * k.beta2 + (k.one_minus_b2 * gg) * gg;
+    const float denom = sqrtf(v) * k.inv_sqrt_bc2 + k.eps;
+    p = p - k.lr_over_bc1 * (m / denom);
+}
+
+__device__ __forceinline__ double powi(double b, int t) {
+    double r = 1.0;
+    while (t > 0) {
+        if (t & 1) r *= b;
+        b *= b;
+        t >>= 1;
+    }
+    return r;
+}
+
+__device__ __forceinline__ uint32_t adam_key(float lr, float b1, float b2) {
+    return __float_as_uint(lr) ^ (__float_as_uint(b1) * 3u) ^ (__float_as_uint(b2) * 7u);
+}
+
+__device__ __forceinline__ uint32_t* adam_next_scalars(uint32_t* ticket, uint32_t gi) { return ticket + 16u * 33u + 4u * gi; }
+__device__ __forceinline__ const uint32_t* adam_next_scalars(const uint32_t* ticket, uint32_t gi) { return ticket + 16u * 33u + 4u * gi; }
+
+__device__ __forceinline__ void adam_step_scalars(const int32_t* step_dev, const uint32_t* nexth, float lr, float beta1,
+                                                  float beta2, float& h0, float& h1) {
+    const int t = step_dev[0] + 1;
+    const uint32_t tag = nexth[0];
+    const float n0 = __uint_as_float(nexth[1]), n1 = __uint_as_float(nexth[2]);
+    if (tag == (uint32_t)t && nexth[3] == adam_key(lr, beta1, beta2)) {
+        h0 = n0, h1 = n1;
+    } else {
+        const double bc1 = 1.0 - powi((double)beta1, t);
+        const double bc2 = 1.0 - powi((double)beta2, t);
+        h0 = (float)((double)lr / bc1), h1 = (float)(1.0 / sqrt(bc2));
+    }
+}
+
+__device__ __forceinline__ AdamK adam_make(float h0, float h1, float beta1, float beta2, float eps, float wd) {
+    AdamK k;
+    k.lr_over_bc1 = h0, k.inv_sqrt_bc2 = h1;
+    k.beta1 = beta1, k.beta2 = beta2;
+    k.one_minus_b1 = (float)(1.0 - (double)beta1), k.one_minus_b2 = (float)(1.0 - (double)beta2);
+    k.eps = eps, k.wd = wd, k.dev_hyper = nullptr;
+    return k;
+}
+
+}
diff --git a/mipsfusion_amd/csrc/elementwise.hip b/mipsfusion_amd/csrc/elementwise.hip
--- a/mipsfusion_amd/csrc/elementwise.hip
+++ b/mipsfusion_amd/csrc/elementwise.hip
@@ -1,4 +1,5 @@
 #include "common.h"
+#include "adam_dev.h"
 
 namespace mipsf {
 
@@ -51,19 +52,6 @@
     if (t >= n3) return;
     const int d = (int)(t % 3);
     dpts[t] = (float)(((double)dxn[t] / nc.norm_factor) / nc.div[d]);
-}
-
-struct AdamK {
-    float lr_over_bc1, beta1, beta2, one_minus_b1, one_minus_b2, inv_sqrt_bc2, eps, wd;
-    const float* dev_hyper;
-};
-
-__device__ __forceinline__ AdamK resolve(AdamK k) {
-    if (k.dev_hyper) {
-        k.lr_over_bc1 = k.dev_hyper[0];
-        k.inv_sqrt_bc2 = k.dev_hyper[1];
-    }
-    return k;
 }
 
 __global__ void adam_advance_kernel(int* __restrict__ step, float* __restrict__ hyper, float lr, float beta1,
@@ -93,15 +81,6 @@
     const double bc2 = 1.0 - pow((double)a.beta2[i], (double)t);
     a.hyper[i][0] = (float)((double)a.lr[i] / bc1);
     a.hyper[i][1] = (float)(1.0 / sqrt(bc2));
-}
-
-__device__ __forceinline__ void adam1(float& p, float& g, float& m, float& v, const AdamK& k) {
-    float gg = g;
-    if (k.wd != 0.f) gg = gg + k.wd * p;
-    m = m + (gg - m) * k.one_minus_b1;
-    v = v * k.beta2 + (k.one_minus_b2 * gg) * gg;
-    const float denom = sqrtf(v) * k.inv_sqrt_bc2 + k.eps;
-    p = p - k.lr_over_bc1 * (m / denom);
 }
 
 template <bool ZERO>
@@ -189,20 +168,6 @@
     }
 }
 
-__device__ __forceinline__ double powi(double b, int t) {
-    double r = 1.0;
-    while (t > 0) {
-        if (t & 1) r *= b;
-        b *= b;
-        t >>= 1;
-    }
-    return r;
-}
-
-__device__ __forceinline__ uint32_t adam_key(float lr, float b1, float b2) {
-    return __float_as_uint(lr) ^ (__float_as_uint(b1) * 3u) ^ (__float_as_uint(b2) * 7u);
-}
-
 struct AdamAllMap {
     uint32_t blk0[MIPSF_ADAM_MAX_TENSORS + 1];
 };
@@ -226,25 +191,10 @@
     uint64_t i = (uint64_t)b * 256 + threadIdx.x;
     float4 pp, gg, mm, vv;
     if (i < n4) pp = p4[i], gg = g4[i], mm = m4[i], vv = v4[i];
-    uint32_t* nexth = ticket + 16u * 33u + 4u * gi;
-    if (threadIdx.x == 0) {
-        const int t = d.step_dev[gi][0] + 1;
-        const uint32_t tag = nexth[0];
-        const float h0 = __uint_as_float(nexth[1]), h1 = __uint_as_float(nexth[2]);
-        if (tag == (uint32_t)t && nexth[3] == adam_key(d.lr[gi], d.beta1[gi], d.beta2[gi])) {
-            hyp[0] = h0, hyp[1] = h1;
-        } else {
-            const double bc1 = 1.0 - powi((double)d.beta1[gi], t);
-            const double bc2 = 1.0 - powi((double)d.beta2[gi], t);
-            hyp[0] = (float)((double)d.lr[gi] / bc1), hyp[1] = (float)(1.0 / sqrt(bc2));
-        }
-    }
+    if (threadIdx.x == 0)
+        adam_step_scalars(d.step_dev[gi], adam_next_scalars(ticket, gi), d.lr[gi], d.beta1[gi], d.beta2[gi], hyp[0], hyp[1]);
     __syncthreads();
-    AdamK k;
-    k.lr_over_bc1 = hyp[0], k.inv_sqrt_bc2 = hyp[1];
-    k.beta1 = d.beta1[gi], k.beta2 = d.beta2[gi];
-    k.one_minus_b1 = (float)(1.0 - (double)d.beta1[gi]), k.one_minus_b2 = (float)(1.0 - (double)d.beta2[gi]);
-    k.eps = d.eps[gi], k.wd = d.weight_decay[gi], k.dev_hyper = nullptr;
+    const AdamK k = adam_make(hyp[0], hyp[1], d.beta1[gi], d.beta2[gi], d.eps[gi], d.weight_decay[gi]);
     if (threadIdx.x == 0) {
         const uint32_t sub = blockIdx.x & 31u;
         const uint32_t n_sub = (gridDim.x - sub + 31u) / 32u;
@@ -261,7 +211,7 @@
                 const double b1 = (double)d.beta1[q], b2 = (double)d.beta2[q];
                 d.hyper_dev[q][0] = (float)((double)d.lr[q] / (1.0 - powi(b1, t)));
                 d.hyper_dev[q][1] = (float)(1.0 / sqrt(1.0 - powi(b2, t)));
-                uint32_t* nx = ticket + 16u * 33u + 4u * q;
+                uint32_t* nx = adam_next_scalars(ticket, q);
                 nx[1] = __float_as_uint((float)((double)d.lr[q] / (1.0 - powi(b1, t + 1))));
                 nx[2] = __float_as_uint((float)(1.0 / sqrt(1.0 - powi(b2, t + 1))));
                 nx[3] = adam_key(d.lr[q], d.beta1[q], d.beta2[q]);
@@ -439,6 +389,7 @@
     MIPSF_REQUIRE(d, "null descriptor");
     MIPSF_REQUIRE(d->n_groups >= 1 && d->n_groups <= MIPSF_ADAM_MAX_GROUPS, "bad group count %u", d->n_groups);
     MIPSF_REQUIRE(d->n_tensors >= 1 && d->n_tensors <= MIPSF_ADAM_MAX_TENSORS, "bad tensor count %u", d->n_tensors);
+    MIPSF_REQUIRE(d->skip_mask == 0u, "skip_mask 0x%x: only mipsf_adam_step_all leaves tensors alone", d->skip_mask);
     for (uint32_t i = 0; i < d->n_groups; ++i) MIPSF_REQUIRE(d->step_dev[i] && d->hyper_dev[i], "null pointer in group %u", i);
     for (uint32_t i = 0; i < d->n_tensors; ++i) {
         MIPSF_REQUIRE(d->param[i] && d->grad[i] && d->exp_avg[i] && d->exp_avg_sq[i], "null pointer in tensor %u", i);
@@ -454,22 +405,28 @@
     MIPSF_REQUIRE(d->n_groups >= 1 && d->n_groups <= MIPSF_ADAM_MAX_GROUPS, "bad group count %u", d->n_groups);
     MIPSF_REQUIRE(d->n_tensors >= 1 && d->n_tensors <= MIPSF_ADAM_MAX_TENSORS, "bad tensor count %u", d->n_tensors);
     for (uint32_t i = 0; i < d->n_groups; ++i) MIPSF_REQUIRE(d->step_dev[i] && d->hyper_dev[i], "null pointer in group %u", i);
+    const uint32_t skip_mask = d->skip_mask;
     AdamAllMap map;
     const int cus = device_cus();
     if (cus <= 0) return 3;
     const uint64_t budget = (uint64_t)cus * 8;
     uint64_t want_all = 0;
-    for (uint32_t i = 0; i < d->n_tensors; ++i) want_all += ((uint64_t)d->numel[i] / 4 + 255) / 256 + 1;
+    MIPSF_REQUIRE(d->n_tensors >= 32u || (skip_mask >> d->n_tensors) == 0u, "skip_mask 0x%x names tensors beyond the %u of the descriptor",
+                  skip_mask, d->n_tensors);
+    for (uint32_t i = 0; i < d->n_tensors; ++i)
+        if (!(skip_mask >> i & 1u)) want_all += ((uint64_t)d->numel[i] / 4 + 255) / 256 + 1;
     uint32_t blocks = 0;
     for (uint32_t i = 0; i < d->n_tensors; ++i) {
         MIPSF_REQUIRE(d->param[i] && d->grad[i] && d->exp_avg[i] && d->exp_avg_sq[i], "null pointer in tensor %u", i);
         MIPSF_REQUIRE(d->group_of[i] < d->n_groups, "tensor %u: group out of range", i);
         map.blk0[i] = blocks;
+        if (skip_mask >> i & 1u) continue;
         uint64_t want = ((uint64_t)d->numel[i] / 4 + 255) / 256 + 1;
         if (want_all > budget) want = want * budget / want_all;
         blocks += (uint32_t)(want < 1 ? 1 : want);
     }
     for (uint32_t i = d->n_tensors; i <= MIPSF_ADAM_MAX_TENSORS; ++i) map.blk0[i] = blocks;
+    MIPSF_REQUIRE(blocks > 0u, "every tensor is skipped: nobody would advance the step counters");
     if (zero_grad) hipLaunchKernelGGL(adam_all_kernel<true>, dim3(blocks), dim3(256), 0, (hipStream_t)stream, *d, map, ticket);
     else hipLaunchKernelGGL(adam_all_kernel<false>, dim3(blocks), dim3(256), 0, (hipStream_t)stream, *d, map, ticket);
     return check_launch("adam_step_all");
diff --git a/mipsfusion_amd/csrc/hashgrid.hip b/mipsfusion_amd/csrc/hashgrid.hip
--- a/mipsfusion_amd/csrc/hashgrid.hip
+++ b/mipsfusion_amd/csrc/hashgrid.hip
@@ -1,5 +1,6 @@
 #include "common.h"
 #include "launch.h"
+#include "adam_dev.h"
 #include "decoder_layout.h"
 
 namespace mipsf {
@@ -193,6 +194,9 @@
 #endif
 #ifndef MIPSF_SC_RUN
 #define MIPSF_SC_RUN 4
+#endif
+#ifndef MIPSF_SC_FLUSH_UNR
+#define MIPSF_SC_FLUSH_UNR 4
 #endif
 #ifndef MIPSF_SC_SKIP_ZERO
 #define MIPSF_SC_SKIP_ZERO 1
@@ -223,6 +227,24 @@
     uint32_t fold_launch;
     uint32_t w_count, w_arrive, w_first, w_parts, w_nitems, w_items;
     uint64_t w_records, w_partial, w_end;
+};
+
+struct ScatterAdam {
+    float* p;
+    float* m;
+    float* v;
+    const int32_t* step_dev;
+    const uint32_t* nexth;
+    float lr, beta1, beta2, eps, wd;
+    uint32_t keep_grad;
+};
+
+struct ScatterAdamShared {
+    AdamK k;
+    float* p;
+    float* m;
+    float* v;
+    uint32_t keep_grad;
 };
 
 static ScatterPlan make_plan(const GridLevels& g, uint32_t M) {
@@ -622,12 +644,12 @@
     return cur;
 }
 
-template <int LAYOUT>
+template <int LAYOUT, bool FUSED>
 __device__ __forceinline__ void scatter_item(const float* __restrict__ x, const float* __restrict__ dout,
                                              float* __restrict__ dparams, uint32_t M, const GridLevels& g,
                                              const ScatterPlan& plan, uint32_t* __restrict__ ws, uint32_t* __restrict__ cw,
                                              uint32_t* sh_flag, double* __restrict__ acc,
-                                             const uint4 desc, const uint32_t item_index) {
+                                             const uint4 desc, const uint32_t item_index, const ScatterAdamShared* sa) {
     const uint32_t item = desc.x;
     const uint32_t sc_plane1 = plan.max_slice;
     (void)sc_plane1;
@@ -644,11 +666,12 @@
     const uint32_t res = g.res[level];
     const float scale = g.scale[level];
     const uint32_t n_rec_bin = desc.y;
+    const bool has_rec = !FUSED || n_rec_bin != 0u;
     const uint32_t r0 = part * part_of(plan, bin);
     const uint32_t n_rec = n_rec_bin - r0 < part_of(plan, bin) ? n_rec_bin - r0 : part_of(plan, bin);
     const uint32_t* __restrict__ rec = ws + plan.w_records + (size_t)bin * M + r0;
 
-    {
+    if (has_rec) {
 #if MIPSF_SC_PLANAR
         for (uint32_t e = threadIdx.x; e < count; e += SC_BLOCK) acc[SC_ACC0(e)] = 0.0, acc[SC_ACC1(e)] = 0.0;
 #else
@@ -659,7 +682,7 @@
     float2* dst = reinterpret_cast<float2*>(dparams) + off + begin;
     constexpr uint32_t FL = SC_MAX_SLICE / SC_BLOCK;
     float2 cur[FL];
-    if (single && !plan.fresh) {
+    if (!FUSED && single && !plan.fresh) {
 #pragma unroll
         for (uint32_t k = 0; k < FL; ++k) {
             const uint32_t e = threadIdx.x + k * SC_BLOCK;
@@ -853,6 +876,40 @@
     __syncthreads();
 
     auto a2 = [&](uint32_t e) { return make_double2(acc[SC_ACC0(e)], acc[SC_ACC1(e)]); };
+    if constexpr (FUSED) {
+        if (single) {
+            constexpr uint32_t FU = MIPSF_SC_FLUSH_UNR;
+            const AdamK k = sa->k;
+            const bool keep = sa->keep_grad != 0u;
+            float2* pp = reinterpret_cast<float2*>(sa->p) + off + begin;
+            float2* pm = reinterpret_cast<float2*>(sa->m) + off + begin;
+            float2* pv = reinterpret_cast<float2*>(sa->v) + off + begin;
+            for (uint32_t e0 = threadIdx.x; e0 < count; e0 += FU * SC_BLOCK) {
+                float2 p2[FU], m2[FU], v2[FU];
+#pragma unroll
+                for (uint32_t u = 0; u < FU; ++u) {
+                    const uint32_t e = e0 + u * SC_BLOCK;
+                    if (e < count) p2[u] = pp[e], m2[u] = pm[e], v2[u] = pv[e];
+                }
+#pragma unroll
+                for (uint32_t u = 0; u < FU; ++u) {
+                    const uint32_t e = e0 + u * SC_BLOCK;
+                    if (e >= count) break;
+                    float2 gr = make_float2(0.f, 0.f);
+                    if (has_rec) {
+                        const double2 a = a2(e);
+                        gr = make_float2((float)a.x, (float)a.y);
+                    }
+                    float gx = gr.x, gy = gr.y;
+                    adam1(p2[u].x, gx, m2[u].x, v2[u].x, k);
+                    adam1(p2[u].y, gy, m2[u].y, v2[u].y, k);
+                    pp[e] = p2[u], pm[e] = m2[u], pv[e] = v2[u];
+                    if (keep) dst[e] = gr;
+                }
+            }
+            return;
+        }
+    }
     if (single) {
 #pragma unroll
         for (uint32_t k = 0; k < FL; ++k) {
@@ -900,36 +957,62 @@
         __syncthreads();
         if (*sh_flag == 0u) return;
         const float2* p2 = part0 + (size_t)(item_index - part) * SC_MAX_SLICE;
-        for (uint32_t e = threadIdx.x; e < count; e += SC_BLOCK)
-            dst[e] = fold_entry<true>(p2 + e, desc.z, plan.fresh ? make_float2(0.f, 0.f) : dst[e]);
+        if constexpr (FUSED) {
+            const AdamK k = sa->k;
+            const bool keep = sa->keep_grad != 0u;
+            float2* pp = reinterpret_cast<float2*>(sa->p) + off + begin;
+            float2* pm = reinterpret_cast<float2*>(sa->m) + off + begin;
+            float2* pv = reinterpret_cast<float2*>(sa->v) + off + begin;
+            for (uint32_t e = threadIdx.x; e < count; e += SC_BLOCK) {
+                float2 pe = pp[e], me = pm[e], ve = pv[e];
+                const float2 gr = fold_entry<true>(p2 + e, desc.z, make_float2(0.f, 0.f));
+                float gx = gr.x, gy = gr.y;
+                adam1(pe.x, gx, me.x, ve.x, k);
+                adam1(pe.y, gy, me.y, ve.y, k);
+                pp[e] = pe, pm[e] = me, pv[e] = ve;
+                if (keep) dst[e] = gr;
+            }
+        } else {
+            for (uint32_t e = threadIdx.x; e < count; e += SC_BLOCK)
+                dst[e] = fold_entry<true>(p2 + e, desc.z, plan.fresh ? make_float2(0.f, 0.f) : dst[e]);
+        }
         if (threadIdx.x == 0) __hip_atomic_store(&cw[plan.w_arrive + bin], 0u, __ATOMIC_RELAXED, __HIP_MEMORY_SCOPE_AGENT);
     }
 }
 
 
-template <int LAYOUT>
+template <int LAYOUT, bool FUSED>
 __global__ __launch_bounds__(SC_BLOCK) void hashgrid_scatter_persist_kernel(const float* __restrict__ x,
                                                                            const float* __restrict__ dout,
                                                                            float* __restrict__ dparams, uint32_t M,
                                                                            GridLevels g, ScatterPlan plan,
                                                                            uint32_t* __restrict__ ws,
-                                                                           uint32_t* __restrict__ cw) {
+                                                                           uint32_t* __restrict__ cw, ScatterAdam ad) {
     extern __shared__ __attribute__((aligned(16))) double acc[];
     __shared__ uint32_t wtot[16];
     __shared__ uint32_t sh_total, sh_next;
     __shared__ uint4 sh_desc;
+    __shared__ uint32_t wemp[FUSED ? 16 : 1];
+    __shared__ uint32_t sh_empty;
+    __shared__ ScatterAdamShared sh_adam;
     constexpr uint32_t PER = SC_MAX_BINS / SC_BLOCK;
     const uint32_t t = threadIdx.x;
     uint32_t* scnt = reinterpret_cast<uint32_t*>(acc + 2 * (size_t)plan.max_slice);
-    uint32_t litm = 0;
+    uint32_t litm = 0, lemp = 0;
 #pragma unroll
     for (uint32_t k = 0; k < PER; ++k) {
         const uint32_t b = t * PER + k;
         const uint32_t c = b < plan.n_bins ? cw[plan.w_count + b] : 0u;
         if (b < plan.n_bins) scnt[b] = c;
         litm += (c + part_of(plan, b) - 1) / part_of(plan, b);
+        lemp += (FUSED && c == 0u) ? 1u : 0u;
+    }
+    if constexpr (FUSED) {
+        const uint32_t mine = t * PER >= plan.n_bins ? 0u : (plan.n_bins - t * PER < PER ? plan.n_bins - t * PER : PER);
+        lemp -= PER - mine;
     }
     uint32_t oitm;
+    uint32_t oemp = 0;
     {
         uint32_t incl = litm;
 #pragma unroll
@@ -938,11 +1021,26 @@
             incl += (int)(t & 63u) >= d ? v : 0u;
         }
         if ((t & 63u) == 63u) wtot[t >> 6] = incl;
+        uint32_t incl_e = lemp;
+        if constexpr (FUSED) {
+#pragma unroll
+            for (int d = 1; d < 64; d <<= 1) {
+                const uint32_t v = (uint32_t)__shfl_up((int)incl_e, d, 64);
+                incl_e += (int)(t & 63u) >= d ? v : 0u;
+            }
+            if ((t & 63u) == 63u) wemp[t >> 6] = incl_e;
+        }
         __syncthreads();
         uint32_t before = 0;
         for (uint32_t q = 0; q < (t >> 6); ++q) before += wtot[q];
         oitm = before + incl - litm;
         if (t == SC_BLOCK - 1) sh_total = before + incl;
+        if constexpr (FUSED) {
+            uint32_t before_e = 0;
+            for (uint32_t q = 0; q < (t >> 6); ++q) before_e += wemp[q];
+            oemp = before_e + incl_e - lemp;
+            if (t == SC_BLOCK - 1) sh_empty = before_e + incl_e;
+        }
     }
     {
         uint32_t first = oitm;
@@ -954,8 +1052,17 @@
             first += parts;
         }
     }
+    if constexpr (FUSED) {
+        if (threadIdx.x == 0) {
+            float h0, h1;
+            adam_step_scalars(ad.step_dev, ad.nexth, ad.lr, ad.beta1, ad.beta2, h0, h1);
+            sh_adam.k = adam_make(h0, h1, ad.beta1, ad.beta2, ad.eps, ad.wd);
+            sh_adam.p = ad.p, sh_adam.m = ad.m, sh_adam.v = ad.v, sh_adam.keep_grad = ad.keep_grad;
+        }
+    }
     __syncthreads();
-    const uint32_t total = sh_total;
+    const uint32_t with_rec = sh_total;
+    const uint32_t total = FUSED ? with_rec + sh_empty : with_rec;
     if (t == 0) sh_next = __hip_atomic_fetch_add(&cw[plan.w_nitems + 1], 1u, __ATOMIC_RELAXED, __HIP_MEMORY_SCOPE_AGENT);
     __syncthreads();
     if (sh_next == gridDim.x - 1) {
@@ -967,7 +1074,20 @@
         __syncthreads();
         const uint32_t i = sh_next;
         if (i >= total) break;
-        if (i >= oitm && i < oitm + litm) {
+        if (FUSED && i >= with_rec) {
+            const uint32_t j = i - with_rec;
+            if (j >= oemp && j < oemp + lemp) {
+                uint32_t rank = oemp;
+#pragma nounroll
+                for (uint32_t k = 0; k < PER; ++k) {
+                    const uint32_t b = t * PER + k;
+                    if (b >= plan.n_bins) break;
+                    if (scnt[b] != 0u) continue;
+                    if (rank == j) sh_desc = make_uint4(b, 0u, 1u, 0u);
+                    ++rank;
+                }
+            }
+        } else if (i >= oitm && i < oitm + litm) {
             uint32_t first = oitm;
             for (uint32_t k = 0; k < PER; ++k) {
                 const uint32_t b = t * PER + k;
@@ -983,7 +1103,7 @@
 #ifdef MIPSF_SC_TRACE
         const uint64_t tr_t0 = wall_clock64();
 #endif
-        scatter_item<LAYOUT>(x, dout, dparams, M, g, plan, ws, cw, &wtot[0], acc, desc, i);
+        scatter_item<LAYOUT, FUSED>(x, dout, dparams, M, g, plan, ws, cw, &wtot[0], acc, desc, i, &sh_adam);
 #ifdef MIPSF_SC_TRACE
         __syncthreads();
         if (t == 0) {
@@ -1005,9 +1125,10 @@
     }
 }
 
-__global__ __launch_bounds__(256) void hashgrid_scatter_reduce_kernel(float* __restrict__ dparams, GridLevels g,
+template <bool FUSED>
+MIPSF_SINGLE_FP32 __global__ __launch_bounds__(256) void hashgrid_scatter_reduce_kernel(float* __restrict__ dparams, GridLevels g,
                                                                       ScatterPlan plan, const uint32_t* __restrict__ ws,
-                                                                      const uint32_t* __restrict__ cw) {
+                                                                      const uint32_t* __restrict__ cw, ScatterAdam ad) {
     const uint32_t bin = blockIdx.x;
     const uint32_t parts = cw[plan.w_parts + bin];
     if (parts <= 1) return;
@@ -1022,7 +1143,24 @@
     const float2* p2 = reinterpret_cast<const float2*>(reinterpret_cast<const float*>(ws) + plan.w_partial) +
                        (size_t)cw[plan.w_first + bin] * SC_MAX_SLICE + e;
     float2* d = reinterpret_cast<float2*>(dparams) + g.offsets[level] + begin + e;
-    *d = fold_entry<false>(p2, parts, plan.fresh ? make_float2(0.f, 0.f) : *d);
+    if constexpr (FUSED) {
+        const size_t at = (size_t)g.offsets[level] + begin + e;
+        float2* pp = reinterpret_cast<float2*>(ad.p) + at;
+        float2* pm = reinterpret_cast<float2*>(ad.m) + at;
+        float2* pv = reinterpret_cast<float2*>(ad.v) + at;
+        float2 pe = *pp, me = *pm, ve = *pv;
+        float h0, h1;
+        adam_step_scalars(ad.step_dev, ad.nexth, ad.lr, ad.beta1, ad.beta2, h0, h1);
+        const AdamK k = adam_make(h0, h1, ad.beta1, ad.beta2, ad.eps, ad.wd);
+        const float2 gr = fold_entry<false>(p2, parts, make_float2(0.f, 0.f));
+        float gx = gr.x, gy = gr.y;
+        adam1(pe.x, gx, me.x, ve.x, k);
+        adam1(pe.y, gy, me.y, ve.y, k);
+        *pp = pe, *pm = me, *pv = ve;
+        if (ad.keep_grad) *d = gr;
+    } else {
+        *d = fold_entry<false>(p2, parts, plan.fresh ? make_float2(0.f, 0.f) : *d);
+    }
 }
 
 template <int LAYOUT>
@@ -1599,7 +1737,7 @@
 
 static int hashgrid_bwd_impl(const float* x, const float* params, const float* dout, float* dparams, float* dx,
                              float* scratch, uint32_t* counters, uint32_t M, const mipsf_grid_meta* meta, int layout,
-                             bool routed, void* stream, bool fresh = false) {
+                             bool routed, void* stream, bool fresh = false, const ScatterAdam* adam = nullptr) {
     GridLevels g;
     if (int rc = to_levels(meta, g)) return rc;
     if (M == 0) return 0;
@@ -1627,16 +1765,24 @@
         per_cu = per_cu < 1u ? 1u : (per_cu > 2048u / SC_BLOCK ? 2048u / SC_BLOCK : per_cu);
         const uint32_t want = (uint32_t)cus * per_cu;
         const uint32_t blocks = plan.max_items < want ? plan.max_items : want;
+        const ScatterAdam ad = adam ? *adam : ScatterAdam{};
         const int rc = with_layout(layout, [&](auto LAY) {
-            constexpr auto kern = hashgrid_scatter_persist_kernel<LAY.value>;
+            if (adam) {
+                constexpr auto kern = hashgrid_scatter_persist_kernel<LAY.value, true>;
+                if (!grant_lds<kern>(lds_bytes)) return lds_refused(lds_bytes);
+                hipLaunchKernelGGL(kern, dim3(blocks), dim3(SC_BLOCK), lds_bytes, s, x, dout, dparams, M, g, plan, ws, cw, ad);
+                return check_launch("hashgrid_scatter (fused Adam)");
+            }
+            constexpr auto kern = hashgrid_scatter_persist_kernel<LAY.value, false>;
             if (!grant_lds<kern>(lds_bytes)) return lds_refused(lds_bytes);
-            hipLaunchKernelGGL(kern, dim3(blocks), dim3(SC_BLOCK), lds_bytes, s, x, dout, dparams, M, g, plan, ws, cw);
+            hipLaunchKernelGGL(kern, dim3(blocks), dim3(SC_BLOCK), lds_bytes, s, x, dout, dparams, M, g, plan, ws, cw, ad);
             return check_launch("hashgrid_scatter");
         });
         if (rc) return rc;
         if (plan.fold_launch) {
-            hipLaunchKernelGGL(hashgrid_scatter_reduce_kernel, dim3(plan.n_bins, (plan.max_slice + 255) / 256), dim3(256), 0, s,
-                               dparams, g, plan, ws, cw);
+            const dim3 rgrid(plan.n_bins, (plan.max_slice + 255) / 256);
+            if (adam) hipLaunchKernelGGL(hashgrid_scatter_reduce_kernel<true>, rgrid, dim3(256), 0, s, dparams, g, plan, ws, cw, ad);
+            else hipLaunchKernelGGL(hashgrid_scatter_reduce_kernel<false>, rgrid, dim3(256), 0, s, dparams, g, plan, ws, cw, ad);
             if (int e = check_launch("hashgrid_scatter_reduce")) return e;
         }
     }
@@ -1648,8 +1794,28 @@
     MIPSF_REQUIRE(a != nullptr, "null argument block");
     MIPSF_REQUIRE(a->struct_size == sizeof(mipsf_hashgrid_bwd_args), "mipsf_hashgrid_bwd_args: struct_size %u, this library expects %u",
                   a->struct_size, (unsigned)sizeof(mipsf_hashgrid_bwd_args));
-    MIPSF_REQUIRE((a->flags & ~(uint32_t)(MIPSF_HG_DPARAMS_ZERO | MIPSF_HG_ROUTED | MIPSF_HG_DETERMINISTIC)) == 0u,
+    MIPSF_REQUIRE((a->flags & ~(uint32_t)(MIPSF_HG_DPARAMS_ZERO | MIPSF_HG_ROUTED | MIPSF_HG_DETERMINISTIC | MIPSF_HG_FUSED_ADAM |
+                                          MIPSF_HG_KEEP_GRAD)) == 0u,
                   "unknown flags 0x%x", a->flags);
+    MIPSF_REQUIRE(!(a->flags & MIPSF_HG_KEEP_GRAD) || (a->flags & MIPSF_HG_FUSED_ADAM), "MIPSF_HG_KEEP_GRAD without MIPSF_HG_FUSED_ADAM");
+    ScatterAdam ad = {};
+    if (a->flags & MIPSF_HG_FUSED_ADAM) {
+        MIPSF_REQUIRE(a->flags & MIPSF_HG_DPARAMS_ZERO, "MIPSF_HG_FUSED_ADAM without MIPSF_HG_DPARAMS_ZERO: the gradient an entry is "
+                      "stepped with must be this call's alone");
+        MIPSF_REQUIRE(a->dx == nullptr, "MIPSF_HG_FUSED_ADAM with dx: the gather form of dx reads params behind the scatter");
+        MIPSF_REQUIRE(!(a->flags & MIPSF_HG_DETERMINISTIC), "MIPSF_HG_FUSED_ADAM with MIPSF_HG_DETERMINISTIC: the fixed-order scatter "
+                      "has no fused step");
+        MIPSF_REQUIRE(a->dparams != nullptr, "MIPSF_HG_FUSED_ADAM with a frozen grid (dparams NULL)");
+        MIPSF_REQUIRE(a->adam.params_rw && a->adam.exp_avg && a->adam.exp_avg_sq && a->adam.step_dev && a->adam.ticket,
+                      "MIPSF_HG_FUSED_ADAM: null pointer in the adam block");
+        MIPSF_REQUIRE((((uintptr_t)a->adam.params_rw | (uintptr_t)a->adam.exp_avg | (uintptr_t)a->adam.exp_avg_sq) & 7) == 0,
+                      "MIPSF_HG_FUSED_ADAM: the table and its moments must be 8-byte aligned");
+        MIPSF_REQUIRE(a->adam.group < MIPSF_ADAM_MAX_GROUPS, "MIPSF_HG_FUSED_ADAM: group %u out of range", a->adam.group);
+        ad.p = a->adam.params_rw, ad.m = a->adam.exp_avg, ad.v = a->adam.exp_avg_sq;
+        ad.step_dev = a->adam.step_dev, ad.nexth = a->adam.ticket + 16u * 33u + 4u * a->adam.group;
+        ad.lr = a->adam.lr, ad.beta1 = a->adam.beta1, ad.beta2 = a->adam.beta2, ad.eps = a->adam.eps, ad.wd = a->adam.weight_decay;
+        ad.keep_grad = (a->flags & MIPSF_HG_KEEP_GRAD) ? 1u : 0u;
+    }
     if (a->flags & MIPSF_HG_DETERMINISTIC) {
         MIPSF_REQUIRE(!(a->flags & MIPSF_HG_ROUTED), "MIPSF_HG_DETERMINISTIC with MIPSF_HG_ROUTED: the routed scratch belongs to "
                       "the fast scatter; the deterministic path takes its own scratch (MIPSF_SIZE_HASHGRID_DET_SCRATCH)");
@@ -1657,7 +1823,8 @@
                                 (a->flags & MIPSF_HG_DPARAMS_ZERO) != 0u, stream);
     }
     return hashgrid_bwd_impl(a->x, a->params, a->dout, a->dparams, a->dx, a->scratch, a->counters, a->M, a->meta, a->feat_layout,
-                             (a->flags & MIPSF_HG_ROUTED) != 0u, stream, (a->flags & MIPSF_HG_DPARAMS_ZERO) != 0u);
+                             (a->flags & MIPSF_HG_ROUTED) != 0u, stream, (a->flags & MIPSF_HG_DPARAMS_ZERO) != 0u,
+                             (a->flags & MIPSF_HG_FUSED_ADAM) ? &ad : nullptr);
 }
 
 int mipsf_hashgrid_indices(const float* x, uint32_t* idx, uint32_t M, const mipsf_grid_meta* meta, void* stream) {
diff --git a/mipsfusion_amd/model/scene_rep.py b/mipsfusion_amd/model/scene_rep.py
--- a/mipsfusion_amd/model/scene_rep.py
+++ b/mipsfusion_amd/model/scene_rep.py
@@ -7,6 +7,7 @@
 
 from .. import ops
 from .._lib import FEAT_LEVEL_MAJOR
+from ..optim import FusedAdam
 from .decoder import MLP_reg
 from .encodings import get_encoder
 
@@ -131,8 +132,14 @@
             else:
                 dparams = torch.zeros_like(grid_params)
         if need_g:
+            fused = None
+            if (direct and ctx.owner.grid_grad_is_zero_at_backward and not det and ops.FUSE_GRID_ADAM and ctx.prec != "f32"
+                    and not torch.is_grad_enabled()):
+                opt = FusedAdam.of(grid_params)
+                fused = opt.fused_grid_step(grid_params) if opt is not None else None
             ops.hashgrid_bwd(xn, grid_params.detach(), dfeat, dparams, ctx.meta, FEAT_LEVEL_MAJOR, None, routed=ctx.routed,
-                             dparams_zero=(not direct) or fresh_grad or ctx.owner.grid_grad_is_zero_at_backward, deterministic=det)
+                             dparams_zero=(not direct) or fresh_grad or ctx.owner.grid_grad_is_zero_at_backward, deterministic=det,
+                             **({} if fused is None else {"fused_adam": fused}))
             ctx.routed = None
         if need_x:
             ops.hashgrid_dx_from_jac(jac, dfeat, dx, ctx.meta, FEAT_LEVEL_MAJOR, tiles=tiles,
diff --git a/mipsfusion_amd/ops.py b/mipsfusion_amd/ops.py
--- a/mipsfusion_amd/ops.py
+++ b/mipsfusion_amd/ops.py
@@ -179,31 +179,43 @@
 HG_DPARAMS_ZERO = 1
 HG_ROUTED = 2
 HG_DETERMINISTIC = 4
+HG_FUSED_ADAM = 8
+HG_KEEP_GRAD = 16
 _HG_IGNORE_ZERO_HINT = bool(os.environ.get("MIPSF_HG_IGNORE_ZERO_HINT"))
+FUSE_GRID_ADAM = (os.environ.get("MIPSF_FUSED_GRID_ADAM", "0") == "1"
+                  and os.environ.get("MIPSF_NO_FUSED_GRID_ADAM", "0") != "1")
 
 
 def hashgrid_bwd(x, params, dout, dparams, meta, layout=FEAT_AOS, dx: Optional[torch.Tensor] = None, routed=None,
-                 dparams_zero=False, deterministic=False):
+                 dparams_zero=False, deterministic=False, fused_adam=None, keep_grad=False):
     M = x.shape[0]
     if PROFILE is not None:
         global _LAST_SCATTER_DOUT
         _LAST_SCATTER_DOUT = dout
     a = _lib.HashgridBwdArgs.new(M=M, x=dptr(x), params=dptr(params), dout=dptr(dout), dparams=dptr(dparams),
                                  meta=C.pointer(meta), feat_layout=layout)
+    extra = 0
+    if fused_adam is not None:
+        f = fused_adam
+        extra = HG_FUSED_ADAM | (HG_KEEP_GRAD if keep_grad else 0)
+        a.adam.params_rw, a.adam.exp_avg, a.adam.exp_avg_sq = dptr(params), dptr(f["exp_avg"]), dptr(f["exp_avg_sq"])
+        a.adam.step_dev, a.adam.ticket, a.adam.group = dptr(f["step_dev"], torch.int32), dptr(f["ticket"], torch.int32), f["group"]
+        a.adam.lr, a.adam.beta1, a.adam.beta2 = f["lr"], f["beta1"], f["beta2"]
+        a.adam.eps, a.adam.weight_decay = f["eps"], f["weight_decay"]
     if deterministic:
         if routed is not None:
             torch.cuda.current_stream(x.device).wait_event(routed[1])
         n = _lib.buffer_size(_lib.SIZE_HASHGRID_DET_SCRATCH, M, 1 if dx is not None else 0, 0, meta)
         scratch = torch.empty(n, dtype=torch.float32, device=x.device)
         a.dx, a.scratch = dptr(dx), dptr(scratch)
-        a.flags = HG_DETERMINISTIC | (HG_DPARAMS_ZERO if (dparams_zero and not _HG_IGNORE_ZERO_HINT) else 0)
+        a.flags = HG_DETERMINISTIC | (HG_DPARAMS_ZERO if (dparams_zero and not _HG_IGNORE_ZERO_HINT) else 0) | extra
         with _timed("hashgrid_bwd"):
             check(lib().mipsf_hashgrid_bwd(C.byref(a), stream_ptr()), "hashgrid_bwd (deterministic)")
         return
     if routed is not None and dx is None and dparams is not None:
         scratch, ev = routed
         torch.cuda.current_stream(x.device).wait_event(ev)
-        a.scratch, a.flags = dptr(scratch), HG_ROUTED
+        a.scratch, a.flags = dptr(scratch), HG_ROUTED | extra | (HG_DPARAMS_ZERO if (extra and dparams_zero) else 0)
         with _timed("hashgrid_bwd"):
             check(lib().mipsf_hashgrid_bwd(C.byref(a), stream_ptr()), "hashgrid_bwd (routed)")
         return
@@ -211,7 +223,7 @@
     scratch = torch.empty(n, dtype=torch.float32, device=x.device)
     counters = _scatter_counters(x.device, meta)
     a.dx, a.scratch, a.counters = dptr(dx), dptr(scratch), dptr(counters, torch.int32)
-    a.flags = HG_DPARAMS_ZERO if (dparams_zero and not _HG_IGNORE_ZERO_HINT) else 0
+    a.flags = (HG_DPARAMS_ZERO if (dparams_zero and not _HG_IGNORE_ZERO_HINT) else 0) | extra
     with _timed("hashgrid_bwd"):
         check(lib().mipsf_hashgrid_bwd(C.byref(a), stream_ptr()), "hashgrid_bwd")
 
@@ -833,19 +845,22 @@
         check(lib().mipsf_adam_step_small(C.byref(d), 1 if zero_grad else 0, stream_ptr()), "adam_step_small")
 
 
-def adam_step_all(groups, ticket, zero_grad=False):
+def adam_step_all(groups, ticket, zero_grad=False, skip=()):
     d = _lib.AdamSmall()
     d.n_groups = len(groups)
-    ti, dev, big = 0, None, False
+    ti, dev, big, mask = 0, None, False, 0
     for gi, (step_dev, hyper_dev, lr, b1, b2, eps, wd, tensors) in enumerate(groups):
         d.step_dev[gi], d.hyper_dev[gi] = dptr(step_dev, torch.int32), dptr(hyper_dev)
         d.lr[gi], d.beta1[gi], d.beta2[gi], d.eps[gi], d.weight_decay[gi] = lr, b1, b2, eps, wd
         for p, g, m, v in tensors:
             d.param[ti], d.grad[ti], d.exp_avg[ti], d.exp_avg_sq[ti] = dptr(p), dptr(g), dptr(m), dptr(v)
             d.numel[ti], d.group_of[ti] = p.numel(), gi
-            dev, big = p.device, big or p.numel() > (1 << 20)
+            if any(p.data_ptr() == q.data_ptr() for q in skip):
+                mask |= 1 << ti
+            else:
+                dev, big = p.device, big or p.numel() > (1 << 20)
             ti += 1
-    d.n_tensors = ti
+    d.n_tensors, d.skip_mask = ti, mask
     with _timed("adam_step" if big else "adam_step_small"):
         check(lib().mipsf_adam_step_all(C.byref(d), 1 if zero_grad else 0, dptr(ticket, torch.int32), stream_ptr()),
               "adam_step_all")
diff --git a/mipsfusion_amd/optim.py b/mipsfusion_amd/optim.py
--- a/mipsfusion_amd/optim.py
+++ b/mipsfusion_amd/optim.py
@@ -1,11 +1,15 @@
+import os
+import weakref
+
 import torch
 
 from . import _lib, ops
 
 
-import os
-
 _SPLIT_LAUNCHES = os.environ.get("MIPSF_ADAM_SPLIT", "0") == "1"
+
+
+_OWNER = weakref.WeakValueDictionary()
 
 
 class FusedAdam(torch.optim.Optimizer):
@@ -13,6 +17,19 @@
         super().__init__(params, dict(lr=lr, betas=betas, eps=eps, weight_decay=weight_decay))
         self.capturable = capturable
         self._dev = {}
+        self._stepped_in_backward = None
+
+    def add_param_group(self, param_group):
+        super().add_param_group(param_group)
+        for p in self.param_groups[-1]["params"]:
+            _OWNER[id(p)] = self
+
+    @staticmethod
+    def of(p):
+        opt = _OWNER.get(id(p))
+        if opt is None or not any(q is p for g in opt.param_groups for q in g["params"]):
+            return None
+        return opt
 
     def _ensure_state(self, p):
         st = self.state[p]
@@ -22,6 +39,53 @@
             st["exp_avg_sq"] = torch.zeros_like(p, memory_format=torch.contiguous_format)
         return st
 
+    def _live_work(self):
+        work = []
+        for gi, group in enumerate(self.param_groups):
+            live = [p for p in group["params"] if p.grad is not None and p.numel() > 0]
+            if live:
+                work.append((gi, group, live, None))
+        return work
+
+    def _one_launch(self, work):
+        n_t = sum(len(live) for _, _, live, _ in work)
+        return bool(self.capturable and work and not self._all_small(work) and not _SPLIT_LAUNCHES and
+                    len(work) <= _lib.ADAM_MAX_GROUPS and n_t <= _lib.ADAM_MAX_TENSORS and
+                    all(p.numel() < (1 << 32) and p.is_contiguous() for _, _, live, _ in work for p in live))
+
+    def _group_dev(self, gi, device, start):
+        if gi not in self._dev:
+            self._dev[gi] = (torch.full((1,), start, dtype=torch.int32, device=device),
+                             torch.zeros(2, dtype=torch.float32, device=device))
+        return self._dev[gi]
+
+    def _ticket_block(self, device):
+        if getattr(self, "_ticket", None) is None or self._ticket.device != device:
+            self._ticket = torch.zeros(576, dtype=torch.int32, device=device)
+        return self._ticket
+
+    @torch.no_grad()
+    def fused_grid_step(self, p):
+        if not self.capturable or p.grad is None or not p.is_cuda:
+            return None
+        work = self._live_work()
+        at = [i for i, (_, _, live, _) in enumerate(work) if any(q is p for q in live)]
+        if not at or not self._one_launch(work):
+            return None
+        if self._stepped_in_backward is not None:
+            raise RuntimeError("FusedAdam: a second backward found the hash table already stepped by the first one -- "
+                               "grid_grad_is_zero_at_backward promises ONE backward per step(zero_grad=True)")
+        gi, group, live, _ = work[at[0]]
+        steps = {self._ensure_state(q)["step"] for q in live}
+        if len(steps) > 1:
+            return None
+        st = self.state[p]
+        step_dev, _ = self._group_dev(gi, p.device, st["step"])
+        self._stepped_in_backward = (p, at[0])
+        return dict(exp_avg=st["exp_avg"], exp_avg_sq=st["exp_avg_sq"], step_dev=step_dev, ticket=self._ticket_block(p.device),
+                    group=at[0], lr=group["lr"], beta1=group["betas"][0], beta2=group["betas"][1], eps=group["eps"],
+                    weight_decay=group["weight_decay"])
+
     @staticmethod
     def _all_small(work):
         n_t = sum(len(live) for _, _, live, _ in work)
@@ -36,6 +100,7 @@
                 st["step"] = 0
                 tensors += [st["exp_avg"], st["exp_avg_sq"]]
         tensors += [step_dev for step_dev, _ in self._dev.values()]
+        self._stepped_in_backward = None
         by_dtype = {}
         for t in tensors:
             by_dtype.setdefault((t.dtype, t.device), []).append(t)
@@ -87,29 +152,29 @@
                 if len({self.state[p]["step"] for p in live}) > 1:
                     raise RuntimeError(f"capturable FusedAdam: the parameters of group {gi} are at different steps "
                                        "(some had no gradient in an earlier step); use capturable=False for that")
-                if gi not in self._dev:
-                    dev = live[0].device
-                    start = self.state[live[0]]["step"] - 1
-                    self._dev[gi] = (torch.full((1,), start, dtype=torch.int32, device=dev),
-                                     torch.zeros(2, dtype=torch.float32, device=dev))
-                hyper = self._dev[gi][1]
+                hyper = self._group_dev(gi, live[0].device, self.state[live[0]]["step"] - 1)[1]
             work.append((gi, group, live, hyper))
+        stepped, self._stepped_in_backward = self._stepped_in_backward, None
+        if stepped is not None:
+            at = [i for i, (_, _, live, _) in enumerate(work) if any(q is stepped[0] for q in live)]
+            if not zero_grad or not self._one_launch(work) or at != [stepped[1]]:
+                raise RuntimeError("FusedAdam: the hash table was stepped by its backward (grid_grad_is_zero_at_backward promises "
+                                   "one backward, then step(zero_grad=True) of the same parameters); this step() is "
+                                   + ("without zero_grad" if not zero_grad else "not the one-launch step that backward planned for"))
         if self.capturable and work and self._all_small(work):
             ops.adam_step_small([(self._dev[gi][0], self._dev[gi][1], group["lr"], group["betas"][0], group["betas"][1],
                                   group["eps"], group["weight_decay"],
                                   [(p.data, p.grad, self.state[p]["exp_avg"], self.state[p]["exp_avg_sq"]) for p in live])
                                  for gi, group, live, _ in work], zero_grad)
             return loss
-        n_t = sum(len(live) for _, _, live, _ in work)
-        if (self.capturable and work and not _SPLIT_LAUNCHES and len(work) <= _lib.ADAM_MAX_GROUPS and n_t <= _lib.ADAM_MAX_TENSORS and
-                all(p.numel() < (1 << 32) and p.is_contiguous() for _, _, live, _ in work for p in live)):
-            if getattr(self, "_ticket", None) is None or self._ticket.device != work[0][2][0].device:
-                self._ticket = torch.zeros(576, dtype=torch.int32, device=work[0][2][0].device)
+        if self._one_launch(work):
+            ticket = self._ticket_block(work[0][2][0].device)
             try:
                 ops.adam_step_all([(self._dev[gi][0], self._dev[gi][1], group["lr"], group["betas"][0], group["betas"][1],
                                     group["eps"], group["weight_decay"],
                                     [(p.data, p.grad, self.state[p]["exp_avg"], self.state[p]["exp_avg_sq"]) for p in live])
-                                   for gi, group, live, _ in work], self._ticket, zero_grad)
+                                   for gi, group, live, _ in work], ticket, zero_grad,
+                                  skip=() if stepped is None else (stepped[0].data,))
             except RuntimeError:
                 self._ticket = None
                 raise
```
